# HenryHZY/VL-PET

Hardware: AMD Instinct MI355X
Metric: multitask samples/sec (BART-base, r=96) (higher is better)
Workload: dtype bf16

## Files before the change

include/vlpet_hip.h:

```cpp
#ifndef VLPET_HIP_H
#define VLPET_HIP_H
#include <stddef.h>
#include <stdint.h>

#ifdef __cplusplus
extern "C" {
#endif

#define VLPET_F32 0
#define VLPET_BF16 1

#define VLPET_E_SHAPE (-1)
#define VLPET_E_RANK (-2)
#define VLPET_E_ALIGN (-3)
#define VLPET_E_WORKSPACE (-4)
#define VLPET_E_NULL (-5)
#define VLPET_E_DTYPE (-6)
#define VLPET_E_ALIAS (-7)

#define VLPET_GATE_NONE 0
#define VLPET_GATE_MUL 1
#define VLPET_GATE_ADD 2

typedef void* vlpet_stream_t;
// ... 73 lines not shown
                                     float delta_scale, float x2_scale, float gate_scale,
                                     int io_dtype, vlpet_stream_t stream);

int vlpet_adapter_gate_bwd_saved_y(int phases, const void* dy, const void* x1, const void* x2, const void* y, const void* saved,
                                   const void* packed_a, const void* packed_g, const void* dx1_in, void* dx1, void* dx2,
                                   float* dwd, float* dbd, float* dwu, float* dbu,
                                   float* dwgd, float* dbgd, float* dwgu, float* dbgu,
                                   int r, int rg, void* workspace, size_t workspace_bytes,
                                   int64_t M, int d, int tiles, int gate_mode,
                                   float delta_scale, float x2_scale, float gate_scale,
                                   int io_dtype, vlpet_stream_t stream);

int vlpet_parallel_adapter_fwd(const void* x, const void* y, const void* packed, void* out,
                               int64_t M, int d, int tiles, float scale,
                               int io_dtype, vlpet_stream_t stream);
int vlpet_parallel_adapter_bwd(const void* dy, const void* x, const void* packed, void* dx,
                               float* dwd, float* dbd, float* dwu, float* dbu, int r,
                               void* workspace, size_t workspace_bytes,
                               int64_t M, int d, int tiles, float scale,
                               int io_dtype, vlpet_stream_t stream);

int vlpet_parallel_adapter_fwd_save(const void* x, const void* y, const void* packed, void* out, void* saved,
                                    int64_t M, int d, int tiles, float scale, int io_dtype, vlpet_stream_t stream);
int vlpet_parallel_adapter_bwd_saved(const void* dy, const void* x, const void* saved, const void* packed, void* dx,
                                     float* dwd, float* dbd, float* dwu, float* dbu, int r,
                                     void* workspace, size_t workspace_bytes, int64_t M, int d, int tiles,
                                     float scale, int io_dtype, vlpet_stream_t stream);

int vlpet_lora_delta_fwd(const void* x, const void* base, const void* packed,
                         const uint8_t* keep_mask, float p, uint64_t seed, uint8_t* keep_out, void* out,
                         int64_t M, int d, int tiles, float scaling,
                         int io_dtype, vlpet_stream_t stream);
int vlpet_lora_delta_bwd(const void* dy, const void* x, const void* packed,
                         const uint8_t* keep_mask, float p, uint64_t seed, void* dx,
                         float* da, float* db, int r,
                         void* workspace, size_t workspace_bytes,
                         int64_t M, int d, int tiles, float scaling,
                         int io_dtype, vlpet_stream_t stream);

size_t vlpet_lora_saved_bytes(int64_t M, int d, int tiles, int io_dtype);
int vlpet_lora_delta_fwd_save(const void* x, const void* base, const void* packed,
                              const uint8_t* keep_mask, float p, uint64_t seed, uint8_t* keep_out, void* out,
                              void* saved, int64_t M, int d, int tiles, float scaling,
                              int io_dtype, vlpet_stream_t stream);
int vlpet_lora_r8_applies(int64_t M, int d, int r, int io_dtype);
int vlpet_lora_delta_fwd_r8(const void* x, const void* base, const void* packed, const uint8_t* keep_mask, float p,
                            uint64_t seed, uint8_t* keep_out, void* out, void* saved, int64_t M, int d, int r,
                            float scaling, int io_dtype, vlpet_stream_t stream);
int vlpet_lora_delta_bwd_saved(const void* dy, const void* x, const void* saved, const void* packed,
                               const uint8_t* keep_mask, float p, uint64_t seed, void* dx,
                               float* da, float* db, int r,
                               void* workspace, size_t workspace_bytes,
                               int64_t M, int d, int tiles, float scaling,
                               int io_dtype, vlpet_stream_t stream);

size_t vlpet_visproj_packed_bytes(int d_out, int feat_dim, int io_dtype);
int vlpet_visproj_pack(const void* w, const void* b, int d_out, int feat_dim, int param_dtype, int io_dtype,
                       void* packed, vlpet_stream_t stream);
int vlpet_visproj_fwd(const void* feats, const void* packed, const float* gamma, const float* beta,
                      const void* r, void* out, void* xhat, float* rstd,
                      int64_t M, int feat_dim, int d_out, float eps, int rms,
                      int io_dtype, vlpet_stream_t stream);
size_t vlpet_visproj_gemm_workspace_bytes(int64_t M, int feat_dim, int d_out);
size_t vlpet_visproj_gemm_exchange_bytes(int d_out);
int vlpet_visproj_fwd_gemm(const void* feats, const void* w_io, const float* bias, const float* gamma, const float* beta,
                           const void* r, void* out, void* xhat, float* rstd, float* mean, void* workspace,
                           size_t workspace_bytes, int64_t M, int feat_dim, int d_out, float eps, int rms, int io_dtype,
                           vlpet_stream_t stream);
int vlpet_visproj_fwd_gemm_cfg(const void* feats, const void* w_io, const float* bias, const float* gamma, const float* beta,
                               const void* r, void* out, void* xhat, float* rstd, float* mean, void* workspace,
                               size_t workspace_bytes, int64_t M, int feat_dim, int d_out, float eps, int rms, int io_dtype,
                               int form, int rows_per_workgroup, vlpet_stream_t stream);
int vlpet_sum_n(const void* const* srcs, int n, void* out, int64_t len, int io_dtype, vlpet_stream_t stream);
int vlpet_vispos_applies(int d, int n_img);
int vlpet_vispos_fwd(const float* pos, const float* w, const float* b, const float* gamma, const float* beta,
                     const void* img_table, int img_table_dtype, int n_img, const int64_t* img_ids, int64_t img_ids_bstride,
                     const void* obj_table, int obj_table_dtype, int64_t obj_rows, const int64_t* obj_ids, int64_t obj_ids_bstride,
                     void* out, int64_t M, int N, int d, float eps, int rms, int io_dtype, vlpet_stream_t stream);
size_t vlpet_vispos_bwd_workspace_bytes(int64_t M, int d, int n_img);
int vlpet_vispos_bwd(const void* dout, const float* pos, const float* w, const float* b, const float* gamma,
                     int n_img, const int64_t* img_ids, int64_t img_ids_bstride,
                     float* dw, float* db, float* dgamma, float* dbeta, float* dimg,
                     void* workspace, size_t workspace_bytes, int64_t M, int N, int d, float eps, int rms, int io_dtype,
                     vlpet_stream_t stream);
size_t vlpet_visproj_wgrad_workspace_bytes(int64_t M, int feat_dim, int d_out);
size_t vlpet_visproj_wgrad_workspace_bytes_io(int64_t M, int feat_dim, int d_out, int io_dtype);
int vlpet_visproj_wgrad(const void* dpre, const void* feats, float* dw, float* db,
                        void* workspace, size_t workspace_bytes,
                        int64_t M, int feat_dim, int d_out, int io_dtype, vlpet_stream_t stream);

size_t vlpet_lowrank_packed_bytes(int tiles, int feat_dim, int d_out, int io_dtype);
int vlpet_lowrank_pack(const void* const* wd_heads, const void* const* bd_heads, int n_heads,
                       const void* wu, const void* bu, int r, int feat_dim, int d_out, int tiles,
                       int param_dtype, int io_dtype, void* packed, vlpet_stream_t stream);
int vlpet_lowrank_gate_fwd(const void* feats, const void* packed_a, const void* packed_g, void* fe,
                           void* saved, int64_t M, int feat_dim, int d_out, int tiles, int gate_residual,
                           int io_dtype, vlpet_stream_t stream);
size_t vlpet_lowrank_bwd_workspace_bytes(int64_t M, int feat_dim, int d_out, int tiles, int io_dtype);
int vlpet_lowrank_gate_bwd(const void* dfe, const void* feats, const void* saved, const void* packed_a,
                           const void* packed_g, float* dwd, float* dbd, float* dwu, float* dbu,
                           float* dwgd, float* dbgd, float* dwgu, float* dbgu, int r, int rg,
                           void* workspace, size_t workspace_bytes, int64_t M, int feat_dim, int d_out,
                           int tiles, int gate_residual, int io_dtype, vlpet_stream_t stream);
int vlpet_norm_residual_fwd(const void* y, const void* r, const float* gamma, const float* beta, void* out,
                            float* mean, float* rstd, int64_t M, int d, float eps, int io_dtype,
                            vlpet_stream_t stream);

int vlpet_sublayer_tail_partials(int64_t M);
int vlpet_sublayer_tail_fwd(const void* y, const void* x1, const float* gamma, const float* beta, void* out,
                            void* h_save, float* mean, float* rstd, uint8_t* keep_out, int64_t M, int d,
                            float eps, float p, uint64_t seed, int norm_mode, int io_dtype,
                            vlpet_stream_t stream);
int vlpet_sublayer_tail_bwd(const void* dout, const void* h_save, const float* mean, const float* rstd,
                            const float* gamma, void* dx1, void* dy, float* dgb_partials, int64_t M, int d,
                            float p, uint64_t seed, int norm_mode, int io_dtype, vlpet_stream_t stream);
int vlpet_sublayer_tail_bwd_out(const void* dout, const void* out_save, const float* rstd, const float* gamma, const float* beta,
                                void* dx1, void* dy, float* dgb_partials, int64_t M, int d,
                                float p, uint64_t seed, int io_dtype, vlpet_stream_t stream);
int vlpet_sublayer_tail_reduce(const float* dgb_partials, int n_partials, int d, float* dgamma, float* dbeta,
                               vlpet_stream_t stream);
int vlpet_colsum_partial(const void* x, int64_t M, int n, float* workspace, int io_dtype, vlpet_stream_t stream);
int vlpet_reduce_batch(const float* const* partials, float* const* out0, float* const* out1, const int* n_partials,
                       const int* d, int n_jobs, vlpet_stream_t stream);
int vlpet_rmsnorm_fwd(const void* x, const float* gamma, void* out, float* rstd, int64_t M, int d, float eps, int io_dtype,
                      vlpet_stream_t stream);
int vlpet_rmsnorm_bwd(const void* dout, const void* x, const float* rstd, const float* gamma, const void* dx_in, void* dx,
                      float* dgb_partials, int64_t M, int d, int io_dtype, vlpet_stream_t stream);
int vlpet_sublayer_tail_rms_fwd(const void* y, const void* x1, const float* gamma_next, void* sum, void* normed, float* rstd,
                                int64_t M, int d, float eps, float p, uint64_t seed, int io_dtype, vlpet_stream_t stream);
int vlpet_rmsnorm_tail_bwd(const void* d_normed, const void* sum, const float* rstd, const float* gamma_next, const void* dsum_in,
                           void* dx1, void* dy, float* dgb_partials, int64_t M, int d, float p, uint64_t seed, int io_dtype,
                           vlpet_stream_t stream);
int vlpet_colsum(const void* x, int64_t M, int n, float* workspace, float* out, int io_dtype, vlpet_stream_t stream);
int vlpet_layernorm_bwd_xhat(const void* dout, const void* xhat, const float* rstd, const float* gamma, void* dx,
                             float* dgb_partials, int64_t M, int d, int io_dtype, vlpet_stream_t stream);

#define VLPET_ACT_GELU 0
#define VLPET_ACT_GELU_NEW 1
#define VLPET_ACT_RELU 2
int vlpet_act_dropout_fwd(const void* x, void* out, uint8_t* keep_out, int64_t n, int act, float p, uint64_t seed,
                          int io_dtype, vlpet_stream_t stream);
int vlpet_act_dropout_bwd(const void* dy, const void* x, void* dx, int64_t n, int act, float p, uint64_t seed,
                          int io_dtype, vlpet_stream_t stream);
int vlpet_concat_dropout_fwd(const void* a, const void* v, void* x, int64_t B, int La, int Lv, int d, float p, uint64_t seed,
                             int io_dtype, vlpet_stream_t stream);
int vlpet_concat_dropout_bwd(const void* dx, void* da, void* dv, int64_t B, int La, int Lv, int d, float p, uint64_t seed,
                             int io_dtype, vlpet_stream_t stream);
int vlpet_prefix_concat_chunks(int64_t B);
size_t vlpet_prefix_concat_ws_bytes(int64_t B, int P, int d);
int vlpet_prefix_concat_dropout_fwd(const void* pre, const void* a, const void* v, void* x, int64_t B, int P, int La, int Lv, int d,
                                    float p, uint64_t seed, int io_dtype, vlpet_stream_t stream);
int vlpet_prefix_concat_dropout_bwd(const void* dx, void* dpre, void* da, void* dv, float* ws, int64_t B, int P, int La, int Lv, int d,
                                    float p, uint64_t seed, int io_dtype, vlpet_stream_t stream);

int vlpet_ce_loss_fwd(const void* logits, const int64_t* labels, float* loss, float* lse, int64_t N, int V, int ld,
                      int io_dtype, vlpet_stream_t stream);
int vlpet_ce_loss_bwd(const void* logits, const int64_t* labels, const float* lse, const float* dloss, void* dlogits,
                      int64_t N, int V, int ld, int io_dtype, vlpet_stream_t stream);
int vlpet_ce_loss_fwd_checked(const void* logits, const int64_t* labels, float* loss, float* lse, unsigned int* bad_count,
                              int64_t N, int V, int ld, int io_dtype, vlpet_stream_t stream);

#define VLPET_ATTN_MAX_LEN 128
int vlpet_attn_fwd(const void* q, const void* k, const void* v, const uint8_t* key_mask, void* o, float* lse, uint8_t* keep_out,
                   int B, int H, int Lq, int Lk, int causal, float scale, float p, uint64_t seed, vlpet_stream_t stream);
int vlpet_attn_bwd(const void* q, const void* k, const void* v, const void* o, const void* dout, const float* lse,
                   const uint8_t* key_mask, void* dq, void* dk, void* dv, int B, int H, int Lq, int Lk, int causal,
                   float scale, float p, uint64_t seed, vlpet_stream_t stream);
int vlpet_attn_fwd_ld(const void* q, const void* k, const void* v, const uint8_t* key_mask, void* o, float* lse, uint8_t* keep_out,
                      int B, int H, int Lq, int Lk, int ld_q, int ld_kv, int causal, float scale, float p, uint64_t seed,
                      vlpet_stream_t stream);
int vlpet_attn_bwd_ld(const void* q, const void* k, const void* v, const void* o, const void* dout, const float* lse,
                      const uint8_t* key_mask, void* dq, void* dk, void* dv, int B, int H, int Lq, int Lk, int ld_q, int ld_kv,
                      int causal, float scale, float p, uint64_t seed, vlpet_stream_t stream);
int vlpet_attn_fwd_bias(const void* q, const void* k, const void* v, const uint8_t* key_mask, const float* bias, void* o,
                        float* lse, uint8_t* keep_out, int B, int H, int Lq, int Lk, int ld_q, int ld_kv, int causal,
                        float scale, float p, uint64_t seed, vlpet_stream_t stream);
int vlpet_attn_bwd_bias(const void* q, const void* k, const void* v, const void* o, const void* dout, const float* lse,
                        const uint8_t* key_mask, const float* bias, const float* bias_t, void* dq, void* dk, void* dv,
                        int B, int H, int Lq, int Lk, int ld_q, int ld_kv, int causal, float scale, float p, uint64_t seed,
                        vlpet_stream_t stream);
int vlpet_attn_fwd_kv(const void* q, const void* k, const void* v, const uint8_t* key_mask, const float* bias, void* o,
                      float* lse, uint8_t* keep_out, int B, int H, int Lq, int Lk, int ld_q, int ld_k, int ld_v, int causal,
                      float scale, float p, uint64_t seed, vlpet_stream_t stream);
int vlpet_attn_bwd_kv(const void* q, const void* k, const void* v, const void* o, const void* dout, const float* lse,
                      const uint8_t* key_mask, const float* bias, const float* bias_t, void* dq, void* dk, void* dv,
                      int B, int H, int Lq, int Lk, int ld_q, int ld_k, int ld_v, int causal, float scale, float p, uint64_t seed,
                      vlpet_stream_t stream);
#define VLPET_ATTN_LONG_MAX_LEN 1024
int vlpet_attn_long_fwd(const void* q, const void* k, const void* v, const uint8_t* key_mask, const float* bias, void* o,
                        float* lse, int B, int H, int Lq, int Lk, int ld_q, int ld_k, int ld_v, int causal, float scale,
                        vlpet_stream_t stream);
int vlpet_attn_long_fwd_train(const void* q, const void* k, const void* v, const uint8_t* key_mask, const float* bias, void* o,
                              float* lse, uint8_t* keep_out, int B, int H, int Lq, int Lk, int ld_q, int ld_k, int ld_v, int causal,
                              float scale, float p, uint64_t seed, vlpet_stream_t stream);
int vlpet_attn_long_bwd(const void* q, const void* k, const void* v, const void* o, const void* dout, const float* lse,
                        const uint8_t* key_mask, const float* bias, const float* bias_t, void* dq, void* dk, void* dv,
                        int B, int H, int Lq, int Lk, int ld_q, int ld_k, int ld_v, int causal, float scale, float p, uint64_t seed,
                        float* delta, vlpet_stream_t stream);

int vlpet_downsample_fwd(const void* x, void* out, int64_t n_images, int s_in, int s_out, int dim,
                         int in_dtype, int out_dtype, vlpet_stream_t stream);

int vlpet_rowgate_partials(int64_t M);
int vlpet_row_dot(const void* a, const void* c, const float* wa, const float* wc, float* s_out, int64_t M, int d,
                  int io_dtype, vlpet_stream_t stream);
int vlpet_row_affine(const void* h, const float* alpha, const float* gamma, void* y, int64_t M, int d,
                     int io_dtype, vlpet_stream_t stream);
int vlpet_rowgate_bwd(const void* dy, const void* x1, const void* h, const float* alpha, const float* beta,
                      const float* wa, const float* wc, void* dh, void* dx1, float* partials, int64_t M, int d,
                      int io_dtype, vlpet_stream_t stream);
int vlpet_vecgate_fwd(const void* h, const float* v, const float* u, void* y, int64_t M, int d, int io_dtype,
                      vlpet_stream_t stream);
int vlpet_vecgate_bwd(const void* dy, const void* h, const float* v, void* dh, float* partials, int64_t M, int d,
                      int io_dtype, vlpet_stream_t stream);

int vlpet_optim_blocks(int64_t n);
int vlpet_grad_sumsq(const float* g, int64_t n, float* partials, vlpet_stream_t stream);
int vlpet_adamw_step(float* p, float* g, float* m, float* v, const uint8_t* decay_mask, int64_t n,
                     const float* partials, int n_partials, float max_norm, float grad_scale, float lr,
                     float beta1, float beta2, float eps, float weight_decay, int step, int variant,
                     int zero_grad, float* norm_out, vlpet_stream_t stream);

int vlpet_adamw_step_sliced(float* p, float* g, float* m, float* v, const uint8_t* decay_mask, int64_t n,
                            const float* partials, int n_partials, float max_norm, float grad_scale, float lr,
                            float beta1, float beta2, float eps, float weight_decay, const int32_t* slice_of,
                            const float* slice_bc, int variant, int zero_grad, float* norm_out,
                            vlpet_stream_t stream);

int vlpet_attn_decode(const void* q, int64_t ld_q, void* k_cache, void* v_cache, int64_t ld_k, int64_t bs_k, int64_t ld_v,
                      int64_t bs_v, const void* k_new, const void* v_new, int64_t ld_new, int pos, const uint8_t* key_mask,
                      int64_t ld_mask, const float* bias, int64_t ld_bias, void* o, int64_t ld_o, int B, int H, int D, int Lk,
                      float scale, int io_dtype, vlpet_stream_t stream);
int vlpet_greedy_pick(const void* logits, int64_t ld, int V, int64_t* ids, int64_t ld_ids, int pos, int* unfinished, int* counter,
                      int B, int eos_token_id, int pad_token_id, int min_length, int no_repeat_ngram_size, int io_dtype,
                      vlpet_stream_t stream);

int vlpet_attn_decode_beam(const void* q, int64_t ld_q, void* k_cache, void* v_cache, int64_t ld_k, int64_t bs_k, int64_t ld_v,
                           int64_t bs_v, const void* k_new, const void* v_new, int64_t ld_new, int pos, const uint8_t* key_mask,
                           int64_t ld_mask, const float* bias, int64_t ld_bias, void* o, int64_t ld_o, int B, int H, int D,
                           int Lk, float scale, int group, const int* key_rows, int64_t ld_key_rows, int io_dtype,
                           vlpet_stream_t stream);
int vlpet_beam_rows(const void* logits, int64_t ld, int V, const int64_t* ids, int64_t ld_ids, int pos, int rows, int num_beams,
                    int slices, int eos_token_id, int min_length, int no_repeat_ngram_size, int force_eos, float* part_stats,
                    float* part_val, int* part_tok, int io_dtype, vlpet_stream_t stream);
int vlpet_beam_advance(const float* part_stats, const float* part_val, const int* part_tok, int slices, int V, int B, int num_beams,
                       float* beam_scores, const int64_t* ids_in, int64_t* ids_out, int64_t ld_ids, const int* key_rows_in,
                       int* key_rows_out, int64_t ld_key_rows, int64_t* next_tokens, float* hyp_score, int* hyp_meta,
                       int64_t* hyp_tokens, int64_t ld_hyp, float* item_worst, int* item_state, int* counter, int pos,
                       int eos_token_id, int pad_token_id, float length_penalty, int early_stopping, vlpet_stream_t stream);

int vlpet_attn_decode_at(const void* q, int64_t ld_q, void* k_cache, void* v_cache, int64_t ld_k, int64_t bs_k, int64_t ld_v,
                         int64_t bs_v, const void* k_new, const void* v_new, int64_t ld_new, const int* pos_dev, int pos_limit,
                         const uint8_t* key_mask, int64_t ld_mask, const float* bias, int64_t ld_bias, int64_t pos_stride_bias,
                         void* o, int64_t ld_o, int B, int H, int D, int Lk, float scale, const int* key_rows,
                         int64_t ld_key_rows, int64_t parity_stride_key_rows, int io_dtype, vlpet_stream_t stream);
int vlpet_greedy_pick_at(const void* logits, int64_t ld, int V, int64_t* ids, int64_t ld_ids, const int* pos_dev, int pos_limit,
                         int* unfinished, int* counters, int64_t* next_tokens, int B, int eos_token_id, int pad_token_id,
                         int min_length, int no_repeat_ngram_size, int io_dtype, vlpet_stream_t stream);
int vlpet_beam_rows_at(const void* logits, int64_t ld, int V, const int64_t* ids, int64_t ld_ids, int64_t parity_stride_ids,
                       const int* pos_dev, int pos_limit, int rows, int num_beams, int slices, int eos_token_id, int min_length,
                       int no_repeat_ngram_size, int force_eos_pos, float* part_stats, float* part_val, int* part_tok,
                       int io_dtype, vlpet_stream_t stream);
int vlpet_beam_advance_at(const float* part_stats, const float* part_val, const int* part_tok, int slices, int V, int B,
                          int num_beams, float* beam_scores, int64_t* ids, int64_t ld_ids, int64_t parity_stride_ids,
                          int* key_rows, int64_t ld_key_rows, int64_t parity_stride_key_rows, int64_t* next_tokens,
                          float* hyp_score, int* hyp_meta, int64_t* hyp_tokens, int64_t ld_hyp, float* item_worst, int* item_state,
                          int* counters, const int* pos_dev, int pos_limit, int eos_token_id, int pad_token_id,
                          float length_penalty, int early_stopping, vlpet_stream_t stream);

int vlpet_adapter_tail_rows(void);
int vlpet_adapter_tail_applies(int64_t M, int d, int r, int io_dtype);
int vlpet_adapter_tail_fwd(const void* h, const void* res, const void* down_w, const void* down_b, const void* up_w,
                           const void* up_b, const float* gamma, const float* beta, void* out, int64_t M, int d, int r,
                           float scale, float eps, int norm_mode, int param_dtype, int io_dtype, vlpet_stream_t stream);

size_t vlpet_phm_workspace_bytes(int d, int r, int n);
int vlpet_phm_expand_pair_fwd(const void* rule_d, const void* W_d, const void* rule_u, const void* W_u, void* wt_d, void* wt_u,
                              int d, int r, int n, int param_dtype, vlpet_stream_t stream);
int vlpet_phm_expand_pair_bwd(const float* dwt_d, const float* dwt_u, const void* rule_d, const void* W_d, const void* rule_u,
                              const void* W_u, float* drule_d, float* dW_d, float* drule_u, float* dW_u, void* workspace,
                              size_t workspace_bytes, int d, int r, int n, int param_dtype, vlpet_stream_t stream);

#ifdef __cplusplus
}
#endif
#endif
```

vl-pet_amd/_lib.py:

```python
from __future__ import annotations

import ctypes
import os
from ctypes import c_char_p, c_float, c_int, c_int64, c_size_t, c_uint64, c_void_p

_HERE = os.path.dirname(os.path.abspath(__file__))
LIB_PATH = os.environ.get("VLPET_LIB") or os.path.join(_HERE, "lib", "libvlpet_hip.so")

VLPET_F32 = 0
VLPET_BF16 = 1
GATE_NONE, GATE_MUL, GATE_ADD = 0, 1, 2

_lib = None

SIGNATURES = {
    "vlpet_version": (c_int, []),
    "vlpet_error_string": (c_char_p, [c_int]),
    "vlpet_rank_tiles": (c_int, [c_int]),
    "vlpet_packed_bytes": (c_size_t, [c_int, c_int, c_int]),
    "vlpet_pack_pair": (c_int, [c_void_p, c_void_p, c_int, c_void_p, c_void_p, c_int, c_int, c_int, c_int, c_int,
                                c_void_p, c_void_p]),
    "vlpet_pack_pairs": (c_int, [c_int, c_void_p, c_void_p, c_int, c_void_p, c_void_p, c_int, c_int, c_int, c_int, c_int,
                                 c_void_p, c_void_p]),
    "vlpet_adapter_gate_fwd": (c_int, [c_void_p, c_void_p, c_void_p, c_void_p, c_void_p, c_int64, c_int, c_int,
                                       c_int, c_float, c_float, c_float, c_int, c_void_p]),
    "vlpet_saved_bytes": (c_size_t, [c_int64, c_int, c_int]),
    "vlpet_adapter_gate_fwd_save": (c_int, [c_void_p, c_void_p, c_void_p, c_void_p, c_void_p, c_void_p, c_int64, c_int,
                                            c_int, c_int, c_float, c_float, c_float, c_int, c_void_p]),
    "vlpet_adapter_gate_bwd_saved": (c_int, [c_int] + [c_void_p] * 8 + [c_void_p] * 8 + [c_int, c_int, c_void_p, c_size_t,
                                                                                        c_int64, c_int, c_int, c_int,
                                                                                        c_float, c_float, c_float, c_int,
                                                                                        c_void_p]),
    "vlpet_adapter_gate_bwd_saved_acc": (c_int, [c_int] + [c_void_p] * 9 + [c_void_p] * 8 + [c_int, c_int, c_void_p, c_size_t,
                                                                                            c_int64, c_int, c_int, c_int,
                                                                                            c_float, c_float, c_float, c_int,
                                                                                            c_void_p]),
    "vlpet_adapter_gate_bwd_saved_y": (c_int, [c_int] + [c_void_p] * 10 + [c_void_p] * 8 + [c_int, c_int, c_void_p, c_size_t,
                                                                                           c_int64, c_int, c_int, c_int,
                                                                                           c_float, c_float, c_float, c_int,
                                                                                           c_void_p]),
    "vlpet_bwd_workspace_bytes": (c_size_t, [c_int64, c_int, c_int, c_int, c_int]),
    "vlpet_adapter_gate_bwd_form": (c_int, [c_int64, c_int, c_int, c_int]),
    "vlpet_adapter_gate_bwd_finalize_launch": (c_int, [c_int64, c_int, c_int, c_int]),
    "vlpet_debug_build": (c_int, []),
    "vlpet_test_hold_cus": (c_int, [c_int, c_int, c_void_p, c_int, c_void_p]),
    "vlpet_set_seed_counter": (c_int, [c_void_p]),
    "vlpet_adapter_gate_bwd": (c_int, [c_void_p] * 7 + [c_void_p] * 8 + [c_int, c_int, c_void_p, c_size_t, c_int64,
                                                                         c_int, c_int, c_int, c_float, c_float,
                                                                         c_float, c_int, c_void_p]),
    "vlpet_adapter_gate_bwd_phase": (c_int, [c_int] + [c_void_p] * 7 + [c_void_p] * 8 + [c_int, c_int, c_void_p, c_size_t,
                                                                                        c_int64, c_int, c_int, c_int,
                                                                                        c_float, c_float, c_float, c_int,
                                                                                        c_void_p]),
    "vlpet_parallel_adapter_fwd": (c_int, [c_void_p, c_void_p, c_void_p, c_void_p, c_int64, c_int, c_int, c_float,
                                           c_int, c_void_p]),
    "vlpet_parallel_adapter_bwd": (c_int, [c_void_p] * 4 + [c_void_p] * 4 + [c_int, c_void_p, c_size_t, c_int64,
                                                                             c_int, c_int, c_float, c_int, c_void_p]),
    "vlpet_parallel_adapter_fwd_save": (c_int, [c_void_p, c_void_p, c_void_p, c_void_p, c_void_p, c_int64, c_int, c_int,
                                                c_float, c_int, c_void_p]),
    "vlpet_parallel_adapter_bwd_saved": (c_int, [c_void_p] * 5 + [c_void_p] * 4 + [c_int, c_void_p, c_size_t, c_int64,
                                                                                   c_int, c_int, c_float, c_int, c_void_p]),
    "vlpet_lora_delta_fwd": (c_int, [c_void_p, c_void_p, c_void_p, c_void_p, c_float, c_uint64, c_void_p, c_void_p,
                                     c_int64, c_int, c_int, c_float, c_int, c_void_p]),
    "vlpet_lora_saved_bytes": (c_size_t, [c_int64, c_int, c_int, c_int]),
    "vlpet_lora_delta_fwd_save": (c_int, [c_void_p, c_void_p, c_void_p, c_void_p, c_float, c_uint64, c_void_p, c_void_p,
                                          c_void_p, c_int64, c_int, c_int, c_float, c_int, c_void_p]),
    "vlpet_lora_r8_applies": (c_int, [c_int64, c_int, c_int, c_int]),
    "vlpet_lora_delta_fwd_r8": (c_int, [c_void_p, c_void_p, c_void_p, c_void_p, c_float, c_uint64, c_void_p, c_void_p,
                                        c_void_p, c_int64, c_int, c_int, c_float, c_int, c_void_p]),
    "vlpet_lora_delta_bwd_saved": (c_int, [c_void_p, c_void_p, c_void_p, c_void_p, c_void_p, c_float, c_uint64, c_void_p,
                                           c_void_p, c_void_p, c_int, c_void_p, c_size_t, c_int64, c_int, c_int, c_float,
                                           c_int, c_void_p]),
    "vlpet_visproj_packed_bytes": (c_size_t, [c_int, c_int, c_int]),
    "vlpet_visproj_pack": (c_int, [c_void_p, c_void_p, c_int, c_int, c_int, c_int, c_void_p, c_void_p]),
    "vlpet_visproj_fwd": (c_int, [c_void_p] * 8 + [c_int64, c_int, c_int, c_float, c_int, c_int, c_void_p]),
    "vlpet_visproj_gemm_workspace_bytes": (c_size_t, [c_int64, c_int, c_int]),
    "vlpet_visproj_gemm_exchange_bytes": (c_size_t, [c_int]),
    "vlpet_visproj_fwd_gemm": (c_int, [c_void_p] * 11 + [c_size_t, c_int64, c_int, c_int, c_float, c_int, c_int, c_void_p]),
    "vlpet_visproj_fwd_gemm_cfg": (c_int, [c_void_p] * 11 + [c_size_t, c_int64, c_int, c_int, c_float, c_int, c_int, c_int, c_int, c_void_p]),
    "vlpet_sum_n": (c_int, [c_void_p, c_int, c_void_p, c_int64, c_int, c_void_p]),
    "vlpet_vispos_applies": (c_int, [c_int, c_int]),
    "vlpet_vispos_fwd": (c_int, [c_void_p] * 5 + [c_void_p, c_int, c_int, c_void_p, c_int64] + [c_void_p, c_int, c_int64, c_void_p, c_int64]
                         + [c_void_p, c_int64, c_int, c_int, c_float, c_int, c_int, c_void_p]),
    "vlpet_vispos_bwd_workspace_bytes": (c_size_t, [c_int64, c_int, c_int]),
    "vlpet_vispos_bwd": (c_int, [c_void_p] * 5 + [c_int, c_void_p, c_int64] + [c_void_p] * 5
                         + [c_void_p, c_size_t, c_int64, c_int, c_int, c_float, c_int, c_int, c_void_p]),
    "vlpet_visproj_wgrad_workspace_bytes": (c_size_t, [c_int64, c_int, c_int]),
    "vlpet_visproj_wgrad_workspace_bytes_io": (c_size_t, [c_int64, c_int, c_int, c_int]),
    "vlpet_visproj_wgrad": (c_int, [c_void_p] * 5 + [c_size_t, c_int64, c_int, c_int, c_int, c_void_p]),
    "vlpet_lowrank_packed_bytes": (c_size_t, [c_int, c_int, c_int, c_int]),
    "vlpet_lowrank_pack": (c_int, [c_void_p, c_void_p, c_int, c_void_p, c_void_p] + [c_int] * 6 + [c_void_p, c_void_p]),
    "vlpet_lowrank_gate_fwd": (c_int, [c_void_p] * 5 + [c_int64] + [c_int] * 5 + [c_void_p]),
    "vlpet_lowrank_bwd_workspace_bytes": (c_size_t, [c_int64, c_int, c_int, c_int, c_int]),
    "vlpet_lowrank_gate_bwd": (c_int, [c_void_p] * 13 + [c_int, c_int, c_void_p, c_size_t, c_int64] + [c_int] * 5 + [c_void_p]),
    "vlpet_norm_residual_fwd": (c_int, [c_void_p] * 7 + [c_int64, c_int, c_float, c_int, c_void_p]),
    "vlpet_rowgate_partials": (c_int, [c_int64]),
    "vlpet_row_dot": (c_int, [c_void_p] * 5 + [c_int64, c_int, c_int, c_void_p]),
    "vlpet_row_affine": (c_int, [c_void_p] * 4 + [c_int64, c_int, c_int, c_void_p]),
    "vlpet_rowgate_bwd": (c_int, [c_void_p] * 10 + [c_int64, c_int, c_int, c_void_p]),
    "vlpet_vecgate_fwd": (c_int, [c_void_p] * 4 + [c_int64, c_int, c_int, c_void_p]),
    "vlpet_vecgate_bwd": (c_int, [c_void_p] * 5 + [c_int64, c_int, c_int, c_void_p]),
    "vlpet_optim_blocks": (c_int, [c_int64]),
    "vlpet_grad_sumsq": (c_int, [c_void_p, c_int64, c_void_p, c_void_p]),
    "vlpet_adamw_step": (c_int, [c_void_p] * 5 + [c_int64, c_void_p, c_int] + [c_float] * 7 + [c_int, c_int, c_int,
                                                                                           c_void_p, c_void_p]),
    "vlpet_adamw_step_sliced": (c_int, [c_void_p] * 5 + [c_int64, c_void_p, c_int] + [c_float] * 7 + [c_void_p, c_void_p,
                                                                                                  c_int, c_int, c_void_p,
                                                                                                  c_void_p]),
    "vlpet_downsample_fwd": (c_int, [c_void_p, c_void_p, c_int64, c_int, c_int, c_int, c_int, c_int, c_void_p]),
    "vlpet_sublayer_tail_partials": (c_int, [c_int64]),
    "vlpet_sublayer_tail_fwd": (c_int, [c_void_p] * 9 + [c_int64, c_int, c_float, c_float, c_uint64, c_int, c_int, c_void_p]),
    "vlpet_sublayer_tail_bwd": (c_int, [c_void_p] * 8 + [c_int64, c_int, c_float, c_uint64, c_int, c_int, c_void_p]),
    "vlpet_sublayer_tail_bwd_out": (c_int, [c_void_p] * 8 + [c_int64, c_int, c_float, c_uint64, c_int, c_void_p]),
    "vlpet_sublayer_tail_reduce": (c_int, [c_void_p, c_int, c_int, c_void_p, c_void_p, c_void_p]),
    "vlpet_layernorm_bwd_xhat": (c_int, [c_void_p] * 6 + [c_int64, c_int, c_int, c_void_p]),
    "vlpet_colsum": (c_int, [c_void_p, c_int64, c_int, c_void_p, c_void_p, c_int, c_void_p]),
    "vlpet_colsum_partial": (c_int, [c_void_p, c_int64, c_int, c_void_p, c_int, c_void_p]),
    "vlpet_reduce_batch": (c_int, [c_void_p, c_void_p, c_void_p, c_void_p, c_void_p, c_int, c_void_p]),
    "vlpet_rmsnorm_fwd": (c_int, [c_void_p] * 4 + [c_int64, c_int, c_float, c_int, c_void_p]),
    "vlpet_rmsnorm_bwd": (c_int, [c_void_p] * 7 + [c_int64, c_int, c_int, c_void_p]),
    "vlpet_sublayer_tail_rms_fwd": (c_int, [c_void_p] * 6 + [c_int64, c_int, c_float, c_float, c_uint64, c_int, c_void_p]),
    "vlpet_rmsnorm_tail_bwd": (c_int, [c_void_p] * 8 + [c_int64, c_int, c_float, c_uint64, c_int, c_void_p]),
    "vlpet_attn_fwd": (c_int, [c_void_p] * 7 + [c_int] * 5 + [c_float, c_float, c_uint64, c_void_p]),
    "vlpet_attn_bwd": (c_int, [c_void_p] * 10 + [c_int] * 5 + [c_float, c_float, c_uint64, c_void_p]),
    "vlpet_attn_fwd_ld": (c_int, [c_void_p] * 7 + [c_int] * 7 + [c_float, c_float, c_uint64, c_void_p]),
    "vlpet_attn_bwd_ld": (c_int, [c_void_p] * 10 + [c_int] * 7 + [c_float, c_float, c_uint64, c_void_p]),
    "vlpet_attn_fwd_bias": (c_int, [c_void_p] * 8 + [c_int] * 7 + [c_float, c_float, c_uint64, c_void_p]),
    "vlpet_attn_bwd_bias": (c_int, [c_void_p] * 12 + [c_int] * 7 + [c_float, c_float, c_uint64, c_void_p]),
    "vlpet_concat_dropout_fwd": (c_int, [c_void_p] * 3 + [c_int64, c_int, c_int, c_int, c_float, c_uint64, c_int, c_void_p]),
    "vlpet_concat_dropout_bwd": (c_int, [c_void_p] * 3 + [c_int64, c_int, c_int, c_int, c_float, c_uint64, c_int, c_void_p]),
    "vlpet_prefix_concat_chunks": (c_int, [c_int64]),
    "vlpet_prefix_concat_ws_bytes": (c_size_t, [c_int64, c_int, c_int]),
    "vlpet_prefix_concat_dropout_fwd": (c_int, [c_void_p] * 4 + [c_int64, c_int, c_int, c_int, c_int, c_float, c_uint64, c_int, c_void_p]),
    "vlpet_prefix_concat_dropout_bwd": (c_int, [c_void_p] * 5 + [c_int64, c_int, c_int, c_int, c_int, c_float, c_uint64, c_int, c_void_p]),
    "vlpet_attn_fwd_kv": (c_int, [c_void_p] * 8 + [c_int] * 8 + [c_float, c_float, c_uint64, c_void_p]),
    "vlpet_attn_bwd_kv": (c_int, [c_void_p] * 12 + [c_int] * 8 + [c_float, c_float, c_uint64, c_void_p]),
    "vlpet_attn_long_fwd": (c_int, [c_void_p] * 7 + [c_int] * 8 + [c_float, c_void_p]),
    "vlpet_attn_long_fwd_train": (c_int, [c_void_p] * 8 + [c_int] * 8 + [c_float, c_float, c_uint64, c_void_p]),
    "vlpet_attn_long_bwd": (c_int, [c_void_p] * 12 + [c_int] * 8 + [c_float, c_float, c_uint64, c_void_p, c_void_p]),
    "vlpet_ce_loss_fwd": (c_int, [c_void_p] * 4 + [c_int64, c_int, c_int, c_int, c_void_p]),
    "vlpet_ce_loss_fwd_checked": (c_int, [c_void_p] * 5 + [c_int64, c_int, c_int, c_int, c_void_p]),
    "vlpet_ce_loss_bwd": (c_int, [c_void_p] * 5 + [c_int64, c_int, c_int, c_int, c_void_p]),
    "vlpet_act_dropout_fwd": (c_int, [c_void_p] * 3 + [c_int64, c_int, c_float, c_uint64, c_int, c_void_p]),
    "vlpet_act_dropout_bwd": (c_int, [c_void_p] * 3 + [c_int64, c_int, c_float, c_uint64, c_int, c_void_p]),
    "vlpet_attn_decode": (c_int, [c_void_p, c_int64, c_void_p, c_void_p, c_int64, c_int64, c_int64, c_int64, c_void_p, c_void_p,
                                  c_int64, c_int, c_void_p, c_int64, c_void_p, c_int64, c_void_p, c_int64, c_int, c_int, c_int,
                                  c_int, c_float, c_int, c_void_p]),
    "vlpet_greedy_pick": (c_int, [c_void_p, c_int64, c_int, c_void_p, c_int64, c_int, c_void_p, c_void_p, c_int, c_int, c_int,
                                  c_int, c_int, c_int, c_void_p]),
    "vlpet_attn_decode_beam": (c_int, [c_void_p, c_int64, c_void_p, c_void_p, c_int64, c_int64, c_int64, c_int64, c_void_p,
                                       c_void_p, c_int64, c_int, c_void_p, c_int64, c_void_p, c_int64, c_void_p, c_int64, c_int,
                                       c_int, c_int, c_int, c_float, c_int, c_void_p, c_int64, c_int, c_void_p]),
    "vlpet_beam_rows": (c_int, [c_void_p, c_int64, c_int, c_void_p, c_int64, c_int, c_int, c_int, c_int, c_int, c_int, c_int, c_int,
                                c_void_p, c_void_p, c_void_p, c_int, c_void_p]),
    "vlpet_beam_advance": (c_int, [c_void_p, c_void_p, c_void_p, c_int, c_int, c_int, c_int, c_void_p, c_void_p, c_void_p, c_int64,
                                   c_void_p, c_void_p, c_int64, c_void_p, c_void_p, c_void_p, c_void_p, c_int64, c_void_p,
                                   c_void_p, c_void_p, c_int, c_int, c_int, c_float, c_int, c_void_p]),
    "vlpet_attn_decode_at": (c_int, [c_void_p, c_int64, c_void_p, c_void_p, c_int64, c_int64, c_int64, c_int64, c_void_p, c_void_p,
                                     c_int64, c_void_p, c_int, c_void_p, c_int64, c_void_p, c_int64, c_int64, c_void_p, c_int64,
                                     c_int, c_int, c_int, c_int, c_float, c_void_p, c_int64, c_int64, c_int, c_void_p]),
    "vlpet_greedy_pick_at": (c_int, [c_void_p, c_int64, c_int, c_void_p, c_int64, c_void_p, c_int, c_void_p, c_void_p, c_void_p,
                                     c_int, c_int, c_int, c_int, c_int, c_int, c_void_p]),
    "vlpet_beam_rows_at": (c_int, [c_void_p, c_int64, c_int, c_void_p, c_int64, c_int64, c_void_p, c_int, c_int, c_int, c_int, c_int,
                                   c_int, c_int, c_int, c_void_p, c_void_p, c_void_p, c_int, c_void_p]),
    "vlpet_beam_advance_at": (c_int, [c_void_p, c_void_p, c_void_p, c_int, c_int, c_int, c_int, c_void_p, c_void_p, c_int64, c_int64,
                                      c_void_p, c_int64, c_int64, c_void_p, c_void_p, c_void_p, c_void_p, c_int64, c_void_p,
                                      c_void_p, c_void_p, c_void_p, c_int, c_int, c_int, c_float, c_int, c_void_p]),
    "vlpet_adapter_tail_rows": (c_int, []),
    "vlpet_adapter_tail_applies": (c_int, [c_int64, c_int, c_int, c_int]),
    "vlpet_adapter_tail_fwd": (c_int, [c_void_p] * 9 + [c_int64, c_int, c_int, c_float, c_float, c_int, c_int, c_int, c_void_p]),
    "vlpet_lora_delta_bwd": (c_int, [c_void_p, c_void_p, c_void_p, c_void_p, c_float, c_uint64, c_void_p, c_void_p,
                                     c_void_p, c_int, c_void_p, c_size_t, c_int64, c_int, c_int, c_float, c_int,
                                     c_void_p]),
    "vlpet_phm_workspace_bytes": (c_size_t, [c_int, c_int, c_int]),
    "vlpet_phm_expand_pair_fwd": (c_int, [c_void_p] * 6 + [c_int, c_int, c_int, c_int, c_void_p]),
    "vlpet_phm_expand_pair_bwd": (c_int, [c_void_p] * 11 + [c_size_t, c_int, c_int, c_int, c_int, c_void_p]),
}


def load():
    global _lib
    if _lib is not None:
        return _lib
    if not os.path.exists(LIB_PATH):
        raise RuntimeError(
            f"vl-pet_amd: HIP library not found at {LIB_PATH}; run `python -c 'import __graft_entry__ as g; "
            f"g.build()'` (there is no CPU fallback for the PET hot path)")
    import torch
    if torch.cuda.is_available():
        torch.cuda.init()
    lib = ctypes.CDLL(LIB_PATH)
    for name, (res, args) in SIGNATURES.items():
        fn = getattr(lib, name)
        fn.restype = res
        fn.argtypes = args
    _lib = lib
    return lib


def check(code: int, what: str):
    if code != 0:
        msg = load().vlpet_error_string(code)
        raise RuntimeError(f"vl-pet_amd: {what} failed: {msg.decode() if msg else code} (code {code})")
```

vl-pet_amd/csrc/api.hip:

```cpp
#include <atomic>
#include "../../include/vlpet_hip.h"
#include "common.h"
#include "kernels.h"
#include <cmath>
#include <stdlib.h>
#include <stdio.h>
#include <vector>

#define VLPET_VERSION 680
#define VLPET_VERSION_R3 300
#define VLPET_VERSION_R2 221

static inline bool aligned16(const void* p) { return (reinterpret_cast<uintptr_t>(p) & 15) == 0; }
static inline size_t align256(size_t v) { return (v + 255) / 256 * 256; }
static inline int herr(hipError_t e) { return e == hipSuccess ? 0 : (int)e; }

extern "C" int vlpet_version(void) { return VLPET_VERSION; }
extern "C" int vlpet_debug_build(void) { return VLPET_IS_DEBUG_BUILD; }

__global__ __launch_bounds__(64) void hold_cus_kernel(unsigned* release, unsigned long long ticks) {
    extern __shared__ __attribute__((aligned(16))) uint8_t hold_smem[];
    typedef __attribute__((address_space(1))) unsigned gu32;
    if (threadIdx.x == 0) {
        hold_smem[0] = 1;
        const unsigned long long t0 = wall_clock64();
        while (__hip_atomic_load((gu32*)release, __ATOMIC_RELAXED, __HIP_MEMORY_SCOPE_AGENT) == 0u && wall_clock64() - t0 < ticks)
            __builtin_amdgcn_s_sleep(32);
    }
}
extern "C" int vlpet_test_hold_cus(int workgroups, int lds_bytes, void* release_flag, int max_ms, vlpet_stream_t stream) {
    if (!release_flag) return VLPET_E_NULL;
    if (workgroups <= 0 || workgroups > 1024 || lds_bytes < 0 || lds_bytes > 160 * 1024 || max_ms <= 0) return VLPET_E_SHAPE;
    if (max_ms > 10000) max_ms = 10000;
    hipError_t e = hipFuncSetAttribute(reinterpret_cast<const void*>(hold_cus_kernel), hipFuncAttributeMaxDynamicSharedMemorySize, lds_bytes);
    if (e != hipSuccess) return herr(e);
    hipLaunchKernelGGL(hold_cus_kernel, dim3((unsigned)workgroups), dim3(64), (size_t)lds_bytes, (hipStream_t)stream,
                       reinterpret_cast<unsigned*>(release_flag), (unsigned long long)max_ms * 100000ull);
    return herr(hipGetLastError());
}

extern "C" const char* vlpet_error_string(int code) {
    switch (code) {
        case 0: return "success";
        case VLPET_E_SHAPE: return "bad shape (need M > 0, d % 64 == 0, r > 0)";
        case VLPET_E_RANK: return "unsupported bottleneck rank (max 192) or tile count";
        case VLPET_E_ALIGN: return "pointer not 16-byte aligned";
        case VLPET_E_WORKSPACE: return "workspace too small";
        case VLPET_E_NULL: return "required pointer is NULL";
        case VLPET_E_DTYPE: return "unsupported dtype";
        case VLPET_E_ALIAS: return "output overlaps an input";
        default: return code > 0 ? hipGetErrorString((hipError_t)code) : "unknown error";
    }
}

extern "C" int vlpet_rank_tiles(int r) {
    if (r <= 0) return VLPET_E_SHAPE;
    if (r <= 32) return 1;
    if (r <= 96) return 3;
    if (r <= 192) return 6;
    return VLPET_E_RANK;
}

static inline bool tiles_ok(int t) { return t == 1 || t == 3 || t == 6; }
static inline bool dtype_ok(int t) { return t == VLPET_F32 || t == VLPET_BF16; }

extern "C" size_t vlpet_packed_bytes(int tiles, int d, int io_dtype) {
    return (size_t)pack_geom(tiles, d, io_dtype == VLPET_F32 ? 2 : 1).total_bytes;
}

extern "C" int vlpet_pack_pair(const void* const* wd_heads, const void* const* bd_heads, int n_heads,
                               const void* wu, const void* bu, int r, int d, int tiles,
                               int param_dtype, int io_dtype, void* packed, vlpet_stream_t stream) {
    if (!wd_heads || !wu || !packed) return VLPET_E_NULL;
    if (r <= 0 || d <= 0 || d % 64 != 0 || n_heads <= 0 || n_heads > VLPET_MAX_HEADS || r % n_heads != 0)
        return VLPET_E_SHAPE;
    if (!tiles_ok(tiles) || r > 32 * tiles) return VLPET_E_RANK;
    if (!dtype_ok(param_dtype) || !dtype_ok(io_dtype)) return VLPET_E_DTYPE;
    if (!aligned16(packed)) return VLPET_E_ALIGN;
    PackArgs a;
    for (int i = 0; i < VLPET_MAX_HEADS; ++i) {
        a.wd[i] = i < n_heads ? wd_heads[i] : nullptr;
        a.bd[i] = (bd_heads && i < n_heads) ? bd_heads[i] : nullptr;
        if (i < n_heads && a.wd[i] == nullptr) return VLPET_E_NULL;
    }
    a.wu = wu; a.bu = bu;
    a.n_heads = n_heads; a.rows_per_head = r / n_heads;
    a.r = r; a.d = d; a.RT = tiles; a.src_bf16 = param_dtype == VLPET_BF16;
    a.n_packs = 4;
    a.out = reinterpret_cast<uint8_t*>(packed);
    return herr(launch_pack_pair(a, io_dtype == VLPET_F32 ? 2 : 1, (hipStream_t)stream));
}

extern "C" int vlpet_pack_pairs(int n, const void* const* wd_heads_flat, const void* const* bd_heads_flat, int n_heads,
                                const void* const* wu, const void* const* bu, int r, int d, int tiles,
                                int param_dtype, int io_dtype, void* const* packed, vlpet_stream_t stream) {
    if (n <= 0) return 0;
    if (!wd_heads_flat || !wu || !packed) return VLPET_E_NULL;
    if (r <= 0 || d <= 0 || d % 64 != 0 || n_heads <= 0 || n_heads > VLPET_MAX_HEADS || r % n_heads != 0) return VLPET_E_SHAPE;
    if (!tiles_ok(tiles) || r > 32 * tiles) return VLPET_E_RANK;
    if (!dtype_ok(param_dtype) || !dtype_ok(io_dtype)) return VLPET_E_DTYPE;
    for (int i0 = 0; i0 < n; i0 += VLPET_PACK_BATCH) {
        PackBatch b;
        b.n = n - i0 < VLPET_PACK_BATCH ? n - i0 : VLPET_PACK_BATCH;
        for (int k = 0; k < b.n; ++k) {
            PackArgs& a = b.p[k];
            const int idx = i0 + k;
            for (int i = 0; i < VLPET_MAX_HEADS; ++i) {
                a.wd[i] = i < n_heads ? wd_heads_flat[(size_t)idx * n_heads + i] : nullptr;
                a.bd[i] = (bd_heads_flat && i < n_heads) ? bd_heads_flat[(size_t)idx * n_heads + i] : nullptr;
                if (i < n_heads && a.wd[i] == nullptr) return VLPET_E_NULL;
            }
            a.wu = wu[idx]; a.bu = bu ? bu[idx] : nullptr;
            if (!a.wu || !packed[idx]) return VLPET_E_NULL;
            if (!aligned16(packed[idx])) return VLPET_E_ALIGN;
            a.n_heads = n_heads; a.rows_per_head = r / n_heads;
            a.r = r; a.d = d; a.RT = tiles; a.src_bf16 = param_dtype == VLPET_BF16;
            a.n_packs = 4;
            a.out = reinterpret_cast<uint8_t*>(packed[idx]);
        }
        hipError_t e = launch_pack_pairs(b, io_dtype == VLPET_F32 ? 2 : 1, (hipStream_t)stream);
        if (e != hipSuccess) return (int)e;
    }
    return 0;
}

static int check_common(int64_t M, int d, int tiles, int io_dtype) {
    if (M <= 0 || d <= 0 || d % 64 != 0) return VLPET_E_SHAPE;
    if (!tiles_ok(tiles)) return VLPET_E_RANK;
    if (!dtype_ok(io_dtype)) return VLPET_E_DTYPE;
    return 0;
}

static int gate_flags(int gate_mode, int* flags) {
    *flags = 0;
    if (gate_mode == VLPET_GATE_MUL) *flags = PET_GATE;
    else if (gate_mode == VLPET_GATE_ADD) *flags = PET_GATE | PET_GATE_ADD;
    else if (gate_mode != VLPET_GATE_NONE) return VLPET_E_SHAPE;
    return 0;
}

static size_t saved_stride(int64_t M, int tiles, int io_dtype) {
    return align256((size_t)M * 32 * tiles * (io_dtype == VLPET_F32 ? 4 : 2));
}
extern "C" size_t vlpet_saved_bytes(int64_t M, int tiles, int io_dtype) {
    if (M <= 0 || !tiles_ok(tiles)) return 0;
    return 4 * saved_stride(M, tiles, io_dtype);
}

static const DropSpec NO_DROP = {nullptr, nullptr, nullptr, nullptr, 0, 0, 1.f, nullptr};

static std::atomic<const uint64_t*> g_seed_ctr{nullptr};
extern "C" int vlpet_set_seed_counter(const uint64_t* device_counter) {
    g_seed_ctr.store(device_counter);
    return 0;
}

static bool k1_in_launch_reduce(int64_t M) {
    return M >= 8192;
}

static int make_drop(const uint8_t* keep_mask, float p, uint64_t seed, uint8_t* keep_out, DropSpec* ds) {
    if (!(p >= 0.f && p < 1.f)) return VLPET_E_SHAPE;
// ... 1155 lines not shown
                              uint8_t* keep_out, int B, int H, int Lq, int Lk, int causal, float scale, float p, uint64_t seed,
                              vlpet_stream_t stream) {
    return vlpet_attn_fwd_ld(q, k, v, key_mask, o, lse, keep_out, B, H, Lq, Lk, H * 64, H * 64, causal, scale, p, seed, stream);
}

extern "C" int vlpet_attn_bwd_kv(const void* q, const void* k, const void* v, const void* o, const void* dout, const float* lse,
                                 const uint8_t* key_mask, const float* bias, const float* bias_t, void* dq, void* dk, void* dv,
                                 int B, int H, int Lq, int Lk, int ld_q, int ld_k, int ld_v, int causal, float scale, float p, uint64_t seed,
                                 vlpet_stream_t stream) {
    AttnArgs a;
    int rc = attn_args(a, VLPET_ATTN_MAX_LEN, true, q, k, v, key_mask, bias, bias_t, o, lse, nullptr, dout, dq, dk, dv, nullptr,
                       B, H, Lq, Lk, ld_q, ld_k, ld_v, causal, scale, p, seed);
    return rc ? rc : herr(launch_attn(a, true, (hipStream_t)stream));
}
extern "C" int vlpet_attn_bwd_bias(const void* q, const void* k, const void* v, const void* o, const void* dout, const float* lse,
                                   const uint8_t* key_mask, const float* bias, const float* bias_t, void* dq, void* dk, void* dv,
                                   int B, int H, int Lq, int Lk, int ld_q, int ld_kv, int causal, float scale, float p, uint64_t seed,
                                   vlpet_stream_t stream) {
    return vlpet_attn_bwd_kv(q, k, v, o, dout, lse, key_mask, bias, bias_t, dq, dk, dv, B, H, Lq, Lk, ld_q, ld_kv, ld_kv, causal, scale, p, seed,
                             stream);
}

extern "C" int vlpet_attn_bwd_ld(const void* q, const void* k, const void* v, const void* o, const void* dout, const float* lse,
                                 const uint8_t* key_mask, void* dq, void* dk, void* dv, int B, int H, int Lq, int Lk, int ld_q,
                                 int ld_kv, int causal, float scale, float p, uint64_t seed, vlpet_stream_t stream) {
    return vlpet_attn_bwd_bias(q, k, v, o, dout, lse, key_mask, nullptr, nullptr, dq, dk, dv, B, H, Lq, Lk, ld_q, ld_kv, causal, scale, p, seed,
                               stream);
}

extern "C" int vlpet_attn_bwd(const void* q, const void* k, const void* v, const void* o, const void* dout, const float* lse,
                              const uint8_t* key_mask, void* dq, void* dk, void* dv, int B, int H, int Lq, int Lk, int causal,
                              float scale, float p, uint64_t seed, vlpet_stream_t stream) {
    return vlpet_attn_bwd_ld(q, k, v, o, dout, lse, key_mask, dq, dk, dv, B, H, Lq, Lk, H * 64, H * 64, causal, scale, p, seed, stream);
}

static int ce_common(int64_t N, int V, int ld, int io_dtype) {
    if (N <= 0 || V <= 0 || ld < V || (ld & 7) != 0) return VLPET_E_SHAPE;
    if (io_dtype != VLPET_F32 && io_dtype != VLPET_BF16) return VLPET_E_DTYPE;
    return 0;
}

extern "C" int vlpet_ce_loss_fwd_checked(const void* logits, const int64_t* labels, float* loss, float* lse, unsigned int* bad_count,
                                         int64_t N, int V, int ld, int io_dtype, vlpet_stream_t stream) {
    int rc = ce_common(N, V, ld, io_dtype);
    if (rc) return rc;
    if (!logits || !labels || !loss || !lse) return VLPET_E_NULL;
    if (!aligned16(logits)) return VLPET_E_ALIGN;
    CeArgs a{};
    a.logits = logits; a.labels = labels; a.loss = loss; a.lse = lse; a.dloss = nullptr; a.dlogits = nullptr;
    a.N = N; a.V = V; a.ld = ld; a.bad = bad_count;
    return herr(launch_ce(a, false, io_dtype == VLPET_F32, (hipStream_t)stream));
}
extern "C" int vlpet_ce_loss_fwd(const void* logits, const int64_t* labels, float* loss, float* lse, int64_t N, int V, int ld,
                                 int io_dtype, vlpet_stream_t stream) {
    return vlpet_ce_loss_fwd_checked(logits, labels, loss, lse, nullptr, N, V, ld, io_dtype, stream);
}

extern "C" int vlpet_ce_loss_bwd(const void* logits, const int64_t* labels, const float* lse, const float* dloss, void* dlogits,
                                 int64_t N, int V, int ld, int io_dtype, vlpet_stream_t stream) {
    int rc = ce_common(N, V, ld, io_dtype);
    if (rc) return rc;
    if (!logits || !labels || !lse || !dloss || !dlogits) return VLPET_E_NULL;
    if (!aligned16(logits) || !aligned16(dlogits)) return VLPET_E_ALIGN;
    CeArgs a{};
    a.logits = logits; a.labels = labels; a.loss = nullptr; a.lse = const_cast<float*>(lse); a.dloss = dloss; a.dlogits = dlogits;
    a.N = N; a.V = V; a.ld = ld;
    return herr(launch_ce(a, true, io_dtype == VLPET_F32, (hipStream_t)stream));
}

static int act_common(int64_t n, int act, float p, int io_dtype) {
    if (n <= 0 || (n & 7) != 0) return VLPET_E_SHAPE;
    if (act != VLPET_ACT_GELU && act != VLPET_ACT_GELU_NEW && act != VLPET_ACT_RELU) return VLPET_E_SHAPE;
    if (!(p >= 0.0f && p < 1.0f)) return VLPET_E_SHAPE;
    if (io_dtype != VLPET_F32 && io_dtype != VLPET_BF16) return VLPET_E_DTYPE;
    return 0;
}

extern "C" int vlpet_act_dropout_fwd(const void* x, void* out, uint8_t* keep_out, int64_t n, int act, float p, uint64_t seed,
                                     int io_dtype, vlpet_stream_t stream) {
    int rc = act_common(n, act, p, io_dtype);
    if (rc) return rc;
    if (!x || !out) return VLPET_E_NULL;
    if (!aligned16(x) || !aligned16(out)) return VLPET_E_ALIGN;
    ActDropArgs a{};
    a.x = x; a.dy = nullptr; a.out = out; a.keep_out = keep_out; a.n = n; a.act = act; a.thr = tail_thr(p);
    a.keep_scale = a.thr ? 1.0f / (1.0f - p) : 1.0f; a.seed = seed; a.seed_ctr = g_seed_ctr.load();
    return herr(launch_act_dropout(a, false, io_dtype == VLPET_F32, (hipStream_t)stream));
}

extern "C" int vlpet_concat_dropout_fwd(const void* a, const void* v, void* x, int64_t B, int La, int Lv, int d, float p, uint64_t seed,
                                        int io_dtype, vlpet_stream_t stream) {
    if (!a || !v || !x) return VLPET_E_NULL;
    if (B <= 0 || La <= 0 || Lv <= 0 || d <= 0 || d % 8 != 0 || !(p >= 0.f && p < 1.f)) return VLPET_E_SHAPE;
    if (!dtype_ok(io_dtype)) return VLPET_E_DTYPE;
    if (!aligned16(a) || !aligned16(v) || !aligned16(x)) return VLPET_E_ALIGN;
    const uint32_t thr = tail_thr(p);
    return herr(launch_cat_dropout(a, v, x, B, La, Lv, d, thr, thr ? 1.0f / (1.0f - p) : 1.0f, seed, g_seed_ctr.load(), false,
                                   io_dtype == VLPET_F32, (hipStream_t)stream));
}
extern "C" int vlpet_concat_dropout_bwd(const void* dx, void* da, void* dv, int64_t B, int La, int Lv, int d, float p, uint64_t seed,
                                        int io_dtype, vlpet_stream_t stream) {
    if (!dx || (!da && !dv)) return VLPET_E_NULL;
    if (B <= 0 || La <= 0 || Lv <= 0 || d <= 0 || d % 8 != 0 || !(p >= 0.f && p < 1.f)) return VLPET_E_SHAPE;
    if (!dtype_ok(io_dtype)) return VLPET_E_DTYPE;
    if (!aligned16(dx) || (da && !aligned16(da)) || (dv && !aligned16(dv))) return VLPET_E_ALIGN;
    const uint32_t thr = tail_thr(p);
    return herr(launch_cat_dropout(da, dv, const_cast<void*>(dx), B, La, Lv, d, thr, thr ? 1.0f / (1.0f - p) : 1.0f, seed, g_seed_ctr.load(), true,
                                   io_dtype == VLPET_F32, (hipStream_t)stream));
}

extern "C" int vlpet_prefix_concat_chunks(int64_t B) {
    if (B <= 0) return 0;
    int cs, nc;
    prefix_cat_split(B, &cs, &nc);
    return nc;
}
extern "C" size_t vlpet_prefix_concat_ws_bytes(int64_t B, int P, int d) {
    if (B <= 0 || P <= 0 || d <= 0) return 0;
    return (size_t)vlpet_prefix_concat_chunks(B) * (size_t)P * (size_t)d * sizeof(float);
}
static int prefix_cat_common(int64_t B, int P, int La, int Lv, int d, float p, int io_dtype) {
    if (B <= 0 || P <= 0 || La <= 0 || Lv <= 0 || d <= 0 || d % 8 != 0 || !(p >= 0.f && p < 1.f)) return VLPET_E_SHAPE;
    if (!dtype_ok(io_dtype)) return VLPET_E_DTYPE;
    return 0;
}
static PrefixCatArgs prefix_cat_args(const void* pre, const void* a, const void* v, void* x, int64_t B, int P, int La, int Lv, int d, float p,
                                     uint64_t seed) {
    PrefixCatArgs c{};
    c.pre = pre; c.a = a; c.v = v; c.x = x; c.B = B; c.P = P; c.La = La; c.Lv = Lv; c.d = d;
    prefix_cat_split(B, &c.CS, &c.NC);
    c.thr = tail_thr(p); c.keep_scale = c.thr ? 1.0f / (1.0f - p) : 1.0f; c.seed = seed; c.seed_ctr = g_seed_ctr.load();
    return c;
}
extern "C" int vlpet_prefix_concat_dropout_fwd(const void* pre, const void* a, const void* v, void* x, int64_t B, int P, int La, int Lv, int d,
                                               float p, uint64_t seed, int io_dtype, vlpet_stream_t stream) {
    if (!pre || !a || !v || !x) return VLPET_E_NULL;
    if (int rc = prefix_cat_common(B, P, La, Lv, d, p, io_dtype)) return rc;
    if (!aligned16(pre) || !aligned16(a) || !aligned16(v) || !aligned16(x)) return VLPET_E_ALIGN;
    const PrefixCatArgs c = prefix_cat_args(pre, a, v, x, B, P, La, Lv, d, p, seed);
    return herr(launch_prefix_cat(c, false, io_dtype == VLPET_F32, (hipStream_t)stream));
}
extern "C" int vlpet_prefix_concat_dropout_bwd(const void* dx, void* dpre, void* da, void* dv, float* ws, int64_t B, int P, int La, int Lv,
                                               int d, float p, uint64_t seed, int io_dtype, vlpet_stream_t stream) {
    if (!dx || (!dpre && !da && !dv) || (dpre && !ws)) return VLPET_E_NULL;
    if (int rc = prefix_cat_common(B, P, La, Lv, d, p, io_dtype)) return rc;
    if (!dpre && ws) return VLPET_E_SHAPE;
    if (!aligned16(dx) || (dpre && !aligned16(dpre)) || (da && !aligned16(da)) || (dv && !aligned16(dv)) || (ws && !aligned16(ws)))
        return VLPET_E_ALIGN;
    PrefixCatArgs c = prefix_cat_args(nullptr, da, dv, const_cast<void*>(dx), B, P, La, Lv, d, p, seed);
    c.dpre = dpre; c.ws = ws;
    return herr(launch_prefix_cat(c, true, io_dtype == VLPET_F32, (hipStream_t)stream));
}

extern "C" int vlpet_act_dropout_bwd(const void* dy, const void* x, void* dx, int64_t n, int act, float p, uint64_t seed,
                                     int io_dtype, vlpet_stream_t stream) {
    int rc = act_common(n, act, p, io_dtype);
    if (rc) return rc;
    if (!dy || !x || !dx) return VLPET_E_NULL;
    if (!aligned16(dy) || !aligned16(x) || !aligned16(dx)) return VLPET_E_ALIGN;
    ActDropArgs a{};
    a.x = x; a.dy = dy; a.out = dx; a.keep_out = nullptr; a.n = n; a.act = act; a.thr = tail_thr(p);
    a.keep_scale = a.thr ? 1.0f / (1.0f - p) : 1.0f; a.seed = seed; a.seed_ctr = g_seed_ctr.load();
    return herr(launch_act_dropout(a, true, io_dtype == VLPET_F32, (hipStream_t)stream));
}

extern "C" int vlpet_downsample_fwd(const void* x, void* out, int64_t n_images, int s_in, int s_out, int dim,
                                    int in_dtype, int out_dtype, vlpet_stream_t stream) {
    if (!x || !out) return VLPET_E_NULL;
    if (n_images <= 0 || s_in <= 0 || s_out <= 0 || s_out > s_in || dim <= 0 || dim % 8 != 0) return VLPET_E_SHAPE;
    if (!dtype_ok(in_dtype) || !dtype_ok(out_dtype)) return VLPET_E_DTYPE;
    if (!aligned16(x) || !aligned16(out)) return VLPET_E_ALIGN;
    PoolArgs a;
    a.x = x; a.out = out; a.n_img = n_images; a.s_in = s_in; a.s_out = s_out; a.dim = dim;
    return herr(launch_downsample(a, in_dtype == VLPET_F32, out_dtype == VLPET_F32, (hipStream_t)stream));
}

static int row_common(int64_t M, int d, int io_dtype) {
    if (M <= 0 || d <= 0 || d % 8 != 0) return VLPET_E_SHAPE;
    if (!dtype_ok(io_dtype)) return VLPET_E_DTYPE;
    if (d / (io_dtype == VLPET_F32 ? 4 : 8) > 4 * 64) return VLPET_E_SHAPE;
    return 0;
}
static int row_launch(RowArgs& a, int op, int64_t M, int d, int io_dtype, vlpet_stream_t stream) {
    a.M = M; a.d = d;
    return herr(launch_rowgate(a, op, io_dtype == VLPET_F32, (hipStream_t)stream));
}

extern "C" int vlpet_rowgate_partials(int64_t M) { return M > 0 ? rowgate_blocks(M) : 0; }

extern "C" int vlpet_row_dot(const void* a, const void* c, const float* wa, const float* wc, float* s_out, int64_t M,
                             int d, int io_dtype, vlpet_stream_t stream) {
    int rc = row_common(M, d, io_dtype);
    if (rc) return rc;
    if (!a || !s_out) return VLPET_E_NULL;
    if (!wa && !c) return VLPET_E_NULL;
    if (wa && c && !wc) return VLPET_E_NULL;
    if (!aligned16(a) || (c && !aligned16(c))) return VLPET_E_ALIGN;
    RowArgs r{};
    r.a = a; r.c = c; r.va = wa; r.vc = wc; r.rs = s_out;
    return row_launch(r, ROW_DOT, M, d, io_dtype, stream);
}

extern "C" int vlpet_row_affine(const void* h, const float* alpha, const float* gamma, void* y, int64_t M, int d,
                                int io_dtype, vlpet_stream_t stream) {
    int rc = row_common(M, d, io_dtype);
    if (rc) return rc;
    if (!h || !alpha || !y) return VLPET_E_NULL;
    if (!aligned16(h) || !aligned16(y)) return VLPET_E_ALIGN;
    RowArgs r{};
    r.a = h; r.ra = alpha; r.rb = gamma; r.o1 = y;
    return row_launch(r, ROW_AFFINE, M, d, io_dtype, stream);
}

extern "C" int vlpet_rowgate_bwd(const void* dy, const void* x1, const void* h, const float* alpha, const float* beta,
                                 const float* wa, const float* wc, void* dh, void* dx1, float* partials, int64_t M,
                                 int d, int io_dtype, vlpet_stream_t stream) {
    int rc = row_common(M, d, io_dtype);
    if (rc) return rc;
    if (!dy || !x1 || !h || !alpha || !beta || !wa || !wc || !dh || !dx1 || !partials) return VLPET_E_NULL;
    if (!aligned16(dy) || !aligned16(x1) || !aligned16(h) || !aligned16(dh) || !aligned16(dx1)) return VLPET_E_ALIGN;
    RowArgs r{};
    r.a = dy; r.c = x1; r.e = h; r.ra = alpha; r.rb = beta; r.va = wa; r.vc = wc; r.o1 = dh; r.o2 = dx1; r.part = partials;
    return row_launch(r, ROW_BWD, M, d, io_dtype, stream);
}

extern "C" int vlpet_vecgate_fwd(const void* h, const float* v, const float* u, void* y, int64_t M, int d, int io_dtype,
                                 vlpet_stream_t stream) {
    int rc = row_common(M, d, io_dtype);
    if (rc) return rc;
    if (!h || !v || !y) return VLPET_E_NULL;
    if (!aligned16(h) || !aligned16(y)) return VLPET_E_ALIGN;
    RowArgs r{};
    r.a = h; r.va = v; r.vc = u; r.o1 = y;
    return row_launch(r, VEC_FWD, M, d, io_dtype, stream);
}

extern "C" int vlpet_vecgate_bwd(const void* dy, const void* h, const float* v, void* dh, float* partials, int64_t M,
                                 int d, int io_dtype, vlpet_stream_t stream) {
    int rc = row_common(M, d, io_dtype);
    if (rc) return rc;
    if (!dy || !h || !v || !dh || !partials) return VLPET_E_NULL;
    if (!aligned16(dy) || !aligned16(h) || !aligned16(dh)) return VLPET_E_ALIGN;
    RowArgs r{};
    r.a = dy; r.c = h; r.va = v; r.o1 = dh; r.part = partials;
    return row_launch(r, VEC_BWD, M, d, io_dtype, stream);
}

extern "C" int vlpet_optim_blocks(int64_t n) { return n > 0 ? optim_blocks(n) : 0; }

extern "C" int vlpet_grad_sumsq(const float* g, int64_t n, float* partials, vlpet_stream_t stream) {
    if (!g || !partials) return VLPET_E_NULL;
    if (n <= 0) return VLPET_E_SHAPE;
    if (!aligned16(g)) return VLPET_E_ALIGN;
    return herr(launch_sumsq(g, n, partials, (hipStream_t)stream));
}

extern "C" int vlpet_adamw_step(float* p, float* g, float* m, float* v, const uint8_t* decay_mask, int64_t n,
                                const float* partials, int n_partials, float max_norm, float grad_scale, float lr,
                                float beta1, float beta2, float eps, float weight_decay, int step, int variant,
                                int zero_grad, float* norm_out, vlpet_stream_t stream) {
    if (!p || !g || !m || !v || !partials) return VLPET_E_NULL;
    if (n <= 0 || n_partials <= 0 || step <= 0 || (variant != 0 && variant != 1)) return VLPET_E_SHAPE;
    if (!aligned16(p) || !aligned16(g) || !aligned16(m) || !aligned16(v) || (decay_mask && ((uintptr_t)decay_mask & 3)))
        return VLPET_E_ALIGN;
    AdamwArgs a;
    a.p = p; a.g = g; a.m = m; a.v = v; a.decay = decay_mask; a.n = n; a.partials = partials; a.n_partials = n_partials;
    a.max_norm = max_norm; a.grad_scale = grad_scale; a.lr = lr; a.beta1 = beta1; a.beta2 = beta2; a.eps = eps;
    a.weight_decay = weight_decay;
    a.bias_c1 = (float)(1.0 - pow((double)beta1, (double)step));
    a.bias_c2_sqrt = (float)sqrt(1.0 - pow((double)beta2, (double)step));
    a.decay_first = variant == 1; a.eps_scaled = variant == 1; a.zero_grad = zero_grad; a.norm_out = norm_out;
    a.slice_of = nullptr; a.slice_bc = nullptr;
    return herr(launch_adamw(a, (hipStream_t)stream));
}

extern "C" int vlpet_adamw_step_sliced(float* p, float* g, float* m, float* v, const uint8_t* decay_mask, int64_t n,
                                       const float* partials, int n_partials, float max_norm, float grad_scale, float lr,
                                       float beta1, float beta2, float eps, float weight_decay, const int32_t* slice_of,
                                       const float* slice_bc, int variant, int zero_grad, float* norm_out,
                                       vlpet_stream_t stream) {
    if (!p || !g || !m || !v || !partials || !slice_of || !slice_bc) return VLPET_E_NULL;
    if (n <= 0 || n_partials <= 0 || (variant != 0 && variant != 1)) return VLPET_E_SHAPE;
    if (!aligned16(p) || !aligned16(g) || !aligned16(m) || !aligned16(v) || !aligned16(slice_of) ||
        (decay_mask && ((uintptr_t)decay_mask & 3)))
        return VLPET_E_ALIGN;
    AdamwArgs a;
    a.p = p; a.g = g; a.m = m; a.v = v; a.decay = decay_mask; a.n = n; a.partials = partials; a.n_partials = n_partials;
    a.max_norm = max_norm; a.grad_scale = grad_scale; a.lr = lr; a.beta1 = beta1; a.beta2 = beta2; a.eps = eps;
    a.weight_decay = weight_decay; a.bias_c1 = 1.f; a.bias_c2_sqrt = 1.f;
    a.decay_first = variant == 1; a.eps_scaled = variant == 1; a.zero_grad = zero_grad; a.norm_out = norm_out;
    a.slice_of = slice_of; a.slice_bc = slice_bc;
    return herr(launch_adamw(a, (hipStream_t)stream));
}

extern "C" int vlpet_adapter_tail_rows(void) { return adapter_tail_rows(); }

extern "C" int vlpet_adapter_tail_applies(int64_t M, int d, int r, int io_dtype) {
    return (M > 0 && (M + adapter_tail_rows() - 1) / adapter_tail_rows() <= 0x7fffffffLL && adapter_tail_geometry_ok(d, r) && dtype_ok(io_dtype)) ? 1 : 0;
}

static inline bool ranges_overlap(const void* a, const void* b, size_t bytes) {
    const uintptr_t x = reinterpret_cast<uintptr_t>(a), y = reinterpret_cast<uintptr_t>(b);
    return x < y + bytes && y < x + bytes;
}

extern "C" int vlpet_adapter_tail_fwd(const void* h, const void* res, const void* down_w, const void* down_b, const void* up_w,
// ... 82 lines not shown
```

vl-pet_amd/csrc/kernels.h:

```cpp
#pragma once
#include <cstdlib>
#include <hip/hip_runtime.h>
#include <stdint.h>
#include "rng.h"
#include "tuning.h"

#define VLPET_MAX_HEADS 16

struct PackArgs {
    const void* wd[VLPET_MAX_HEADS];
    const void* bd[VLPET_MAX_HEADS];
    const void* wu;
    const void* bu;
    int n_heads, rows_per_head;
    int r, d, RT;
    int src_bf16;
    int n_packs;
    uint8_t* out;
};
hipError_t launch_pack_pair(const PackArgs& a, int NS, hipStream_t stream);
#define VLPET_PACK_BATCH 8
struct PackBatch { PackArgs p[VLPET_PACK_BATCH]; int n; };
hipError_t launch_pack_pairs(const PackBatch& b, int NS, hipStream_t stream);

// ... 200 lines not shown
    int img_tab_bf16, obj_tab_bf16;
    const int64_t* img_ids; const int64_t* obj_ids;
    int64_t img_bstride, obj_bstride;
    int n_img; int64_t obj_rows;
    void* out;
    const void* dout;
    float* partial;
    float* dw; float* db; float* dgamma; float* dbeta; float* dimg;
    int64_t M; int N, d; float eps; int rms;
};
bool vispos_applies(int d, int n_img);
size_t vispos_bwd_workspace_bytes(int64_t M, int d, int n_img);
hipError_t launch_vispos_fwd(const VisPosArgs& a, int io_fp32, hipStream_t stream);
hipError_t launch_vispos_bwd(const VisPosArgs& a, int io_fp32, hipStream_t stream);

struct TailArgs {
    const void* y;
    const void* x1;
    void* out;
    void* h;
    const float* gamma;
    const float* beta;
    float* mean;
    float* rstd;
    uint8_t* keep_out;
    float* dgb;
    int64_t M;
    int d;
    float eps;
    uint32_t thr;
    float keep_scale;
    uint64_t seed;
    const uint64_t* seed_ctr;
    int norm;
    int post;
    int h_xhat;
    int h_out;
    const void* dres;
    int rms;
    void* out2;
    const float* gamma2;
};
hipError_t launch_tail(const TailArgs& a, int io_fp32, bool bwd, hipStream_t stream);
int tail_blocks(int64_t M);

struct Lora8Args {
    const void* x; const void* base; void* out;
    const uint8_t* pk;
    DropSpec drop;
    void* save;
    int64_t M; int d;
    float scaling;
};
bool lora8_applies(int64_t M, int d, int r, int io_fp32);
hipError_t launch_lora8_fwd(const Lora8Args& a, hipStream_t stream);
hipError_t launch_tail_reduce(const float* part, int nb, int d, float* dgamma, float* dbeta, hipStream_t stream);
hipError_t launch_colsum(const void* x, int64_t M, int n, float* part, float* out, int io_fp32, hipStream_t stream);
hipError_t launch_colsum_partial(const void* x, int64_t M, int n, float* part, int io_fp32, hipStream_t stream);
struct ReduceJob { const float* part; float* out0; float* out1; int nb; int d; };
#define VLPET_REDUCE_BATCH 96
struct ReduceBatch { ReduceJob j[VLPET_REDUCE_BATCH]; int n; };
hipError_t launch_tail_reduce_batch(const ReduceBatch& b, int max_d, hipStream_t stream);

struct PoolArgs {
    const void* x;
    void* out;
    int64_t n_img;
    int s_in, s_out, dim;
};
hipError_t launch_downsample(const PoolArgs& a, int in_fp32, int out_fp32, hipStream_t stream);

enum RowOp { ROW_DOT = 0, ROW_AFFINE = 1, ROW_BWD = 2, VEC_FWD = 3, VEC_BWD = 4 };
struct RowArgs {
    const void* a;
    const void* c;
    const void* e;
    void* o1;
    void* o2;
    const float* va;
    const float* vc;
    const float* ra;
    const float* rb;
    float* rs;
    float* part;
    int64_t M;
    int d;
};
hipError_t launch_rowgate(const RowArgs& a, int op, int io_fp32, hipStream_t stream);
int rowgate_blocks(int64_t M);

struct AdamwArgs {
    float* p; float* g; float* m; float* v;
    const uint8_t* decay;
    int64_t n;
    const float* partials; int n_partials;
    float max_norm;
    float grad_scale;
    float lr, beta1, beta2, eps, weight_decay;
    float bias_c1, bias_c2_sqrt;
    int decay_first;
    int eps_scaled;
    int zero_grad;
    float* norm_out;
    const int32_t* slice_of;
    const float* slice_bc;
};
hipError_t launch_add_inplace(void* dst, const void* src, int64_t n, int io_fp32, hipStream_t stream);
struct SumNArgs { const void* src[8]; void* out; };
hipError_t launch_sum_n(const SumNArgs& a, int n, int64_t len, int io_fp32, hipStream_t stream);
hipError_t launch_sumsq(const float* g, int64_t n, float* partials, hipStream_t stream);
hipError_t launch_adamw(const AdamwArgs& a, hipStream_t stream);
int optim_blocks(int64_t n);

inline int pick_row_groups(int64_t M, int max_rg, int min_rg) {
    if (const int rg = vlpet_tuning().rg; rg >= min_rg && rg <= max_rg && rg > 0) return rg;
    int best = max_rg;
    int64_t best_cost = -1;
    for (int rg = max_rg; rg >= min_rg; --rg) {
        const int64_t wgs = (M + 32 * rg - 1) / (32 * rg);
        const int64_t cost = ((wgs + 255) / 256) * (rg + 1);
        if (best_cost < 0 || cost < best_cost) { best = rg; best_cost = cost; }
    }
    return best;
}

#define VLPET_ACT_GELU 0
#define VLPET_ACT_GELU_NEW 1
#define VLPET_ACT_RELU 2
struct ActDropArgs {
    const void* x;
    const void* dy;
    void* out;
    uint8_t* keep_out;
    int64_t n;
    int act;
    uint32_t thr;
    float keep_scale;
    uint64_t seed;
    const uint64_t* seed_ctr;
};
hipError_t launch_act_dropout(const ActDropArgs& a, bool bwd, int io_fp32, hipStream_t stream);
hipError_t launch_cat_dropout(const void* a, const void* v, void* x, int64_t B, int La, int Lv, int d, uint32_t thr, float keep_scale,
                              uint64_t seed, const uint64_t* seed_ctr, bool bwd, int io_fp32, hipStream_t stream);
#define PREFIX_CAT_MAX_CHUNKS 32
struct PrefixCatArgs {
    const void* pre; const void* a; const void* v; void* x;
    void* dpre; float* ws;
    int64_t B; int P, La, Lv, d, CS, NC;
    uint32_t thr; float keep_scale; uint64_t seed; const uint64_t* seed_ctr;
};
void prefix_cat_split(int64_t B, int* cs, int* nc);
hipError_t launch_prefix_cat(const PrefixCatArgs& c, bool bwd, int io_fp32, hipStream_t stream);

struct CeArgs {
    const void* logits;
    const int64_t* labels;
    float* loss;
    float* lse;
    const float* dloss;
    void* dlogits;
    int64_t N;
    int V, ld;
    unsigned int* bad;
};
hipError_t launch_ce(const CeArgs& a, bool bwd, int io_fp32, hipStream_t stream);

struct AttnArgs {
    const __bf16* q; const __bf16* k; const __bf16* v;
    __bf16* o;
    float* lse;
    const __bf16* dout;
    __bf16* dq; __bf16* dk; __bf16* dv;
    const uint8_t* key_mask;
    const float* bias;
    const float* bias_t;
    uint8_t* keep_out;
    int B, H, Lq, Lk, causal;
    int ld_q, ld_kv;
    int ld_v;
    float scale;
    uint32_t thr;
    float inv_keep;
    uint64_t seed;
    const uint64_t* seed_ctr;
    int dbg;
};
size_t attn_lds_bytes(int Lq, int Lk, int bwd);
hipError_t launch_attn(const AttnArgs& a, bool bwd, hipStream_t stream);
hipError_t launch_attn_bwd_fewq(const AttnArgs& a, hipStream_t stream);
hipError_t launch_attn_long_fwd(const AttnArgs& a, hipStream_t stream);
hipError_t launch_attn_long_bwd(const AttnArgs& a, float* delta, hipStream_t stream);

struct AdapterTailArgs {
    const void* h;
    const void* res;
    const void* wd;
    const void* bd;
    const void* wu;
    const void* bu;
    const float* gamma;
    const float* beta;
    void* out;
    int64_t M;
    int d, r;
    float scale, eps;
    int norm;
};
int adapter_tail_rows(void);
bool adapter_tail_geometry_ok(int d, int r);
hipError_t launch_adapter_tail(const AdapterTailArgs& a, int io_fp32, int param_fp32, hipStream_t stream);

struct PhmLayer {
    const void* rule;
    const void* W;
    void* wt;
    const float* dwt;
    float* drule;
    float* dW;
    int in, out;
};
struct PhmArgs {
    PhmLayer l[2];
    int n;
    float* ws;
};
int64_t phm_layer_tiles(int in, int out, int n);
hipError_t launch_phm_expand_fwd(const PhmArgs& a, int param_fp32, hipStream_t stream);
hipError_t launch_phm_expand_bwd(const PhmArgs& a, int param_fp32, hipStream_t stream);
```

vl-pet_amd/host/bart.py:

```python
from __future__ import annotations

import copy
import math
from types import SimpleNamespace

import torch
import torch.nn as nn
import torch.nn.functional as F

from .. import attention as A
from .. import decode as D
from .. import functional as VF
from .. import adapter_tail as AT
from ..adapters import AdapterController
from ..encoder_pet import apply_pet, build_pet, has_pet
from ..lora import LoRALinearController, LoraConfig
from ..visual import Downsample, LowRankVisualEmbedding, VisualEmbedding
from ..prompt import PromptController
from .common import (COMPACTER_DEFAULTS, PROMPT_DEFAULTS, check_sequential_adapter_flags, derived_weights, eval_no_grad, fused_adapter_tail,
                     install_shared_phm_rule, is_key_mask, make_adapter_config, make_prompt_config, sequential_adapters, shift_right, unpack_vis_inputs,
                     value_parallel_adapter)

TASKS = ["vqa", "gqa", "nlvr", "caption"]

# ... 247 lines not shown
                k_slot = None
                if k_pre is not None:
                    (k, k_slot), v = k_pre, VF.linear_acc(src, kv_link, self.v_proj)
                else:
                    k, v = VF.linear_acc(src, kv_link, self.k_proj, self.v_proj)
                if self.attn_value_parallel_adapter is not None:
                    v = self.attn_value_parallel_adapter(src, task, y=v, link=kv_link)
                out = attention_core(q, k, v, self.num_heads, attn_mask, causal, self.dropout, self.training, k_slot=k_slot)
                return _linear(self.out_proj, out)
            v = _linear(self.v_proj, src)
            k = _linear(self.k_proj, src)
        if kv is not None and self.attn_value_parallel_adapter is not None:
            v = self.attn_value_parallel_adapter(src, task, y=v)
        out = attention_core(q, k, v, self.num_heads, attn_mask, causal, self.dropout, self.training)
        return _linear(self.out_proj, out)


    def _step_qkv(self, x, task):
        if self.use_lora:
            return self.q_proj(x, task)[:, 0], _linear(self.k_proj, x)[:, 0], self.v_proj(x, task)[:, 0]
        if FUSE_QKV:
            w, b = self._fused_qkv(x.dtype)
            qkv = F.linear(x[:, 0], w, b)
            E = self.embed_dim
            return qkv[:, :E], qkv[:, E:2 * E], qkv[:, 2 * E:]
        return _linear(self.q_proj, x)[:, 0], _linear(self.k_proj, x)[:, 0], _linear(self.v_proj, x)[:, 0]

    def step_self(self, x, k_cache, v_cache, pos, task=None, key_rows=None, pos_dev=None):
        q, k, v = self._step_qkv(x, task)
        out = D.decode_attention(q, k_cache, v_cache, self.num_heads, pos=pos, k_new=k, v_new=v, scale=self.head_dim ** -0.5,
                                 key_rows=key_rows, pos_dev=pos_dev)
        return _linear(self.out_proj, out[:, None])

    def cross_values(self, enc, task=None):
        v = self.v_proj(enc, task) if self.use_lora else _linear(self.v_proj, enc)
        if self.attn_value_parallel_adapter is not None:
            v = self.attn_value_parallel_adapter(enc, task, y=v)
        return v

    def step_cross(self, x, k_cache, v_cache, key_mask, task=None, group=1):
        q = self.q_proj(x, task) if self.use_lora else _linear(self.q_proj, x)
        out = D.decode_attention(q[:, 0], k_cache, v_cache, self.num_heads, key_mask=key_mask, scale=self.head_dim ** -0.5,
                                 group=group)
        return _linear(self.out_proj, out[:, None])


class BartEncoderLayer(nn.Module):
    def __init__(self, config):
        super().__init__()
        self.config = config
        d = config.d_model
        self.embed_dim = d
        self.self_attn = BartAttention(config, d, config.encoder_attention_heads, config.attention_dropout)
        self.self_attn_layer_norm = HostLayerNorm(d)
        self.dropout, self.activation_dropout = config.dropout, config.activation_dropout
        self.fc1 = nn.Linear(d, config.encoder_ffn_dim)
        self.fc2 = nn.Linear(config.encoder_ffn_dim, d)
        self.final_layer_norm = HostLayerNorm(d)
        build_pet(self, config, d, ("attn", "ff"))
        self.attn_adapter = self.ff_adapter = None
        if sequential_adapters(config, "encoder"):
            self.attn_adapter = AdapterController(config.adapter_config)
            self.ff_adapter = AdapterController(config.adapter_config)
        self.pet_config = copy.copy(config)
        self.pet_config.use_encoder_adapter_scaling = False
        self.pet_config.use_encoder_x2_scaling = False

    def forward(self, hidden, attn_mask=None, task=None):
        residual = hidden
        gl = _new_gemm_link(hidden)
        h = self.self_attn(hidden, attn_mask=attn_mask, task=task, in_link=gl)
        if self.attn_adapter is not None:
            hidden = _adapter_then_tail(self.attn_adapter, task, residual, h, self.self_attn_layer_norm, self.dropout, self.training, gl)
        elif has_pet(self, "attn"):
            hidden = _pet_then_tail(self, "attn", residual, h, self.self_attn_layer_norm, self.dropout, self.training,
                                    self.pet_config, gemm_link=gl)
        else:
            hidden = _tail_linked(residual, h, self.self_attn_layer_norm, self.dropout, self.training, gl)
        residual = hidden
        gl = _new_gemm_link(hidden)
        h = ffn_activation(_first_linear(self.fc1, hidden, gl), "gelu", self.activation_dropout, self.training)
        h = _linear(self.fc2, h)
        if self.ff_adapter is not None:
            return _adapter_then_tail(self.ff_adapter, task, residual, h, self.final_layer_norm, self.dropout, self.training, gl)
        if has_pet(self, "ff"):
            return _pet_then_tail(self, "ff", residual, h, self.final_layer_norm, self.dropout, self.training, self.pet_config,
                                  gemm_link=gl)
        return _tail_linked(residual, h, self.final_layer_norm, self.dropout, self.training, gl)


class BartDecoderLayer(nn.Module):
    def __init__(self, config):
        super().__init__()
        self.config = config
        d = config.d_model
        self.self_attn = BartAttention(config, d, config.decoder_attention_heads, config.attention_dropout)
        self.self_attn_layer_norm = HostLayerNorm(d)
        vpa = bool(config.use_decoder_enc_attn_value_parallel_adapter_down_dim) and not config.use_lora
        self.encoder_attn = BartAttention(config, d, config.decoder_attention_heads, config.attention_dropout,
                                          is_cross=True, value_adapter=vpa)
        self.encoder_attn_layer_norm = HostLayerNorm(d)
        self.dropout, self.activation_dropout = config.dropout, config.activation_dropout
        self.fc1 = nn.Linear(d, config.decoder_ffn_dim)
        self.fc2 = nn.Linear(config.decoder_ffn_dim, d)
        self.final_layer_norm = HostLayerNorm(d)
        self.self_attn_adapter = self.enc_attn_adapter = self.ff_adapter = None
        if sequential_adapters(config, "decoder"):
            self.self_attn_adapter = AdapterController(config.adapter_config)
            if config.add_adapter_cross_attn:
                self.enc_attn_adapter = AdapterController(config.adapter_config)
            self.ff_adapter = AdapterController(config.adapter_config)

    def _tail(self, ctl, task, residual, h, norm, gl=None):
        if ctl is not None:
            return _adapter_then_tail(ctl, task, residual, h, norm, self.dropout, self.training, gl)
        return _tail_linked(residual, h, norm, self.dropout, self.training, gl)

    def forward(self, hidden, enc, enc_mask=None, task=None, k_pre=None):
        residual = hidden
        gl = _new_gemm_link(hidden)
        h = self.self_attn(hidden, causal=True, task=task, in_link=gl)
        hidden = self._tail(self.self_attn_adapter, task, residual, h, self.self_attn_layer_norm, gl)
        residual = hidden
        gl = _new_gemm_link(hidden)
        h = self.encoder_attn(hidden, kv=enc, attn_mask=enc_mask, task=task, in_link=gl, k_pre=k_pre)
        hidden = self._tail(self.enc_attn_adapter, task, residual, h, self.encoder_attn_layer_norm, gl)
        residual = hidden
        gl = _new_gemm_link(hidden)
        h = ffn_activation(_first_linear(self.fc1, hidden, gl), "gelu", self.activation_dropout, self.training)
        h = _linear(self.fc2, h)
        return self._tail(self.ff_adapter, task, residual, h, self.final_layer_norm, gl)


    def step(self, x, cache, pos, state, task=None):
        ks, vs, kx, vx = cache
        kr, pd = state.key_rows, state.pos_dev
        h = self.self_attn.step_self(x, ks, vs, pos, task, key_rows=kr if kr is None or pd is not None else kr[pos & 1], pos_dev=pd)
        x = self._tail(self.self_attn_adapter, task, x, h, self.self_attn_layer_norm)
        h = self.encoder_attn.step_cross(x, kx, vx, state.key_mask, task, group=state.group)
        x = self._tail(self.enc_attn_adapter, task, x, h, self.encoder_attn_layer_norm)
        h = ffn_activation(_linear(self.fc1, x), "gelu", self.activation_dropout, self.training)
        return self._tail(self.ff_adapter, task, x, _linear(self.fc2, h), self.final_layer_norm)


class LearnedPositionalEmbedding(nn.Embedding):

    def __init__(self, num, dim):
        super().__init__(num + 2, dim)

    def forward(self, L: int, device):
        return super().forward(torch.arange(2, L + 2, device=device))


class JointEncoder(nn.Module):
    def __init__(self, config, embed_tokens):
        super().__init__()
        self.config = config
        d = config.d_model
        self.dropout = config.dropout
        self.embed_scale = math.sqrt(d) if config.scale_embedding else 1.0
        self.embed_tokens = embed_tokens
        self.embed_positions = LearnedPositionalEmbedding(config.max_position_embeddings, d)
        self.layers = nn.ModuleList([BartEncoderLayer(config) for _ in range(config.encoder_layers)])
        self.layernorm_embedding = HostLayerNorm(d)
        vis_cls = LowRankVisualEmbedding if getattr(config, "use_lowrank_visual_projector", False) else VisualEmbedding
        self.visual_embedding = vis_cls(config, self.embed_tokens)
        self.downsample = None
        if config.downsample:
            s = int(config.n_boxes ** 0.5)
            self.downsample = Downsample((s, s))
        if getattr(config, "encoder_prompt_config", None) is not None:
            self.prompt_modules = PromptController(config.encoder_prompt_config)

    def forward(self, input_ids, vis_inputs, attention_mask=None, task=None, no_padding=False):
        if getattr(self, "prompt_modules", None) is not None:
            return self._forward_prompted(input_ids, vis_inputs, attention_mask, task, no_padding)
        B, L = input_ids.shape
        if attention_mask is None and not no_padding:
            attention_mask = input_ids.ne(self.config.pad_token_id)
        x = self.embed_tokens(input_ids) * self.embed_scale + self.embed_positions(L, input_ids.device)
        vis = self.visual_embedding(*unpack_vis_inputs(vis_inputs, self.downsample, x.dtype)).to(x.dtype)
        if self.config.share_vis_lang_layer_norm:
            x = self.layernorm_embedding(torch.cat([x, vis], dim=1))
            x = F.dropout(x, p=self.dropout, training=self.training)
        else:
            from ..act import concat_dropout
            x = concat_dropout(self.layernorm_embedding(x), vis, self.dropout, self.training)
        mask = None
        if attention_mask is not None:
            full = torch.cat([attention_mask.bool(), torch.ones(B, vis.shape[1], dtype=torch.bool,
                                                                device=x.device)], dim=1)
            mask = full[:, None, None, :]
        for layer in self.layers:
            x = layer(x, mask, task)
        return x, mask

    def _forward_prompted(self, input_ids, vis_inputs, attention_mask, task, no_padding):
        B, L = input_ids.shape
        if attention_mask is None and not no_padding:
            attention_mask = input_ids.ne(self.config.pad_token_id)
        x = self.embed_tokens(input_ids) * self.embed_scale + self.embed_positions(L, input_ids.device)
        vis = self.visual_embedding(*unpack_vis_inputs(vis_inputs, self.downsample, x.dtype)).to(x.dtype)
        pre = self.prompt_modules.prompt_rows(task).to(x.dtype)
        P = pre.shape[0]
        if self.config.share_vis_lang_layer_norm:
            x = self.layernorm_embedding(torch.cat([pre.expand(B, -1, -1), x, vis], dim=1))
            x = F.dropout(x, p=self.dropout, training=self.training)
        else:
            from ..act import prefix_concat_dropout
            x = prefix_concat_dropout(self.layernorm_embedding(pre), self.layernorm_embedding(x), vis, self.dropout, self.training)
        mask = None
        if attention_mask is not None:
            ones = lambda n: torch.ones(B, n, dtype=torch.bool, device=x.device)
            mask = torch.cat([ones(P), attention_mask.bool(), ones(vis.shape[1])], dim=1)[:, None, None, :]
        for layer in self.layers:
            x = layer(x, mask, task)
        return x, mask


class BartDecoder(nn.Module):
    def __init__(self, config, embed_tokens):
        super().__init__()
        d = config.d_model
        self.dropout = config.dropout
        self.embed_scale = math.sqrt(d) if config.scale_embedding else 1.0
        self.embed_tokens = embed_tokens
        self.embed_positions = LearnedPositionalEmbedding(config.max_position_embeddings, d)
        self.layers = nn.ModuleList([BartDecoderLayer(config) for _ in range(config.decoder_layers)])
        self.layernorm_embedding = HostLayerNorm(d)

    def forward(self, input_ids, enc, enc_mask=None, task=None):
        B, L = input_ids.shape
        x = self.embed_tokens(input_ids) * self.embed_scale + self.embed_positions(L, input_ids.device)
        x = F.dropout(self.layernorm_embedding(x), p=self.dropout, training=self.training)
        n = len(self.layers)
        fused_keys = self._cross_keys_ok(enc, enc_mask)
        encs = VF.fanout(enc, n + (1 if fused_keys else 0))
        ks = self._cross_keys(encs[n]) if fused_keys else None
        for i, (layer, e) in enumerate(zip(self.layers, encs)):
            x = layer(x, e, enc_mask, task, k_pre=None if ks is None else (ks[0][i], None if ks[1] is None else (ks[1], i)))
        return x

    def _cross_keys_ok(self, enc, enc_mask) -> bool:
        if not FUSE_CROSS_KEYS or EAGER_ATTENTION or len(self.layers) < 2 or not enc.is_cuda or enc.dtype != torch.bfloat16:
            return False
        a0 = self.layers[0].encoder_attn
        if _route(enc.shape[1], enc.shape[1], a0.dropout, self.training, grad=True) is None or a0.head_dim != A.HEAD_DIM:
            return False
        if enc_mask is not None and not is_key_mask(enc_mask):
            return False
        return all((not l.encoder_attn.use_lora) and _frozen(l.encoder_attn.k_proj, l.encoder_attn.v_proj) for l in self.layers)

    def _cross_keys(self, enc):
        w, b = derived_weights(self, "_ck_cache", [l.encoder_attn.k_proj for l in self.layers], enc.dtype)
        return VF.cross_key_blocks(enc, w, b, len(self.layers))


    def init_cache(self, enc, key_mask, task, max_length, num_beams=1):
        if FUSE_CROSS_KEYS and not EAGER_ATTENTION and len(self.layers) >= 2 and enc.is_cuda:
            ks = self._cross_keys(enc)[0]
        else:
            ks = [_linear(l.encoder_attn.k_proj, enc) for l in self.layers]
        vs = [l.encoder_attn.cross_values(enc, task) for l in self.layers]
        return D.new_decode_state(enc, enc.shape[2], max_length, ks, vs, key_mask, num_beams)

    def step(self, tok, pos, state, task=None):
        if state.pos_dev is not None:
            p = self.embed_positions.weight[2:].index_select(0, state.pos_dev)
        else:
            p = self.embed_positions.weight[pos + 2]
        x = self.embed_tokens(tok)[:, None] * self.embed_scale + p
        x = F.dropout(self.layernorm_embedding(x), p=self.dropout, training=self.training)
        for layer, c in zip(self.layers, state.layers):
            x = layer.step(x, c, pos, state, task)
        return x[:, 0]


class VLBartModel(nn.Module):
    def __init__(self, config):
        super().__init__()
        self.shared = nn.Embedding(config.vocab_size, config.d_model, padding_idx=config.pad_token_id)
        self.encoder = JointEncoder(config, self.shared)
        self.decoder = BartDecoder(config, self.shared)


shift_tokens_right = shift_right


class VLBart(nn.Module):

    def __init__(self, config):
        super().__init__()
        self.config = config
        self.model = VLBartModel(config)
        self.register_buffer("final_logits_bias", torch.zeros(1, config.vocab_size))
        install_shared_phm_rule(self, [self.model], config.adapter_config)
        self.apply(self._init_weights)
        self.register_load_state_dict_post_hook(lambda module, incompatible: VF.invalidate_caches())

    def _init_weights(self, m):
        std = self.config.init_std
        if isinstance(m, nn.Linear):
            m.weight.data.normal_(0.0, std)
            if m.bias is not None:
                m.bias.data.zero_()
        elif isinstance(m, nn.Embedding):
            m.weight.data.normal_(0.0, std)
            if m.padding_idx is not None:
                m.weight.data[m.padding_idx].zero_()
        if isinstance(m, LoRALinearController):
            for t in m.tasks:
                nn.init.zeros_(m.lora_Bs[t])

    def _logits_bias(self):
        b = self.final_logits_bias
        key = (b.data_ptr(), b._version, VF.FROZEN_EPOCH)
        if getattr(self, "_bias_key", None) != key:
            self._bias_key, self._bias_nonzero = key, bool(b.any())
        return b if self._bias_nonzero else None

    def forward(self, input_ids, vis_inputs, labels, task, attention_mask=None, no_padding=False):
        cfg = self.config
        enc, mask = self.model.encoder(input_ids, vis_inputs, attention_mask, task, no_padding)
        dec_in = shift_tokens_right(labels, cfg.pad_token_id, cfg.decoder_start_token_id)
        h = self.model.decoder(dec_in, enc, mask, task)
        return lm_loss(h, self.model.shared.weight, labels, self._logits_bias())

    def generate(self, input_ids, vis_inputs, task, attention_mask=None, max_length=20, min_length=0, no_repeat_ngram_size=0,
                 eos_token_id=None, pad_token_id=None, no_padding=False, num_beams=1, length_penalty=1.0, early_stopping=False,
                 graph=False):
        from ..lmloss import _padded_head
        cfg = self.config
        eos = getattr(cfg, "eos_token_id", 2) if eos_token_id is None else eos_token_id
        pad = cfg.pad_token_id if pad_token_id is None else pad_token_id
        with eval_no_grad(self):
            enc, mask = self.model.encoder(input_ids, vis_inputs, attention_mask, task, no_padding)
            key_mask = None if mask is None else mask[:, 0, 0, :].contiguous()
            dec = self.model.decoder
            state = dec.init_cache(enc, key_mask, task, max_length, num_beams=int(num_beams))
            V = self.model.shared.weight.shape[0]
            head = _padded_head(self.model.shared.weight, enc.dtype)
            bias = self._logits_bias()

            def make_step(st):
                def step(tok, pos):
                    logits = F.linear(dec.step(tok, pos, st, task), head)
                    if bias is not None:
                        logits[:, :V] += bias[0].to(logits.dtype)
                    return logits
                return step
            if graph:
                gs = D.GenSettings(cfg.decoder_start_token_id, eos, int(pad), int(max_length), int(min_length),
                                   int(no_repeat_ngram_size), int(num_beams), float(length_penalty), bool(early_stopping), True)
                return D.graph_generate(self, state, make_step, V, cfg.decoder_attention_heads, head, gs, key_extra=(task,))[0]
            return D.generate(make_step(state), V, enc.shape[0], enc.device, state.key_rows, cfg.decoder_start_token_id, eos, pad,
                              max_length, min_length, no_repeat_ngram_size, int(num_beams), length_penalty, early_stopping,
                              force_eos=True)
```

vl-pet_amd/lmloss.py:

```python
from __future__ import annotations

from typing import Optional, Tuple

import torch
import torch.nn.functional as F

from . import _lib
from .functional import _io_dtype, _need_cuda, _stream, _timed


def _frozen_epoch():
    from . import functional as _VF
    return _VF.FROZEN_EPOCH


class _CeFn(torch.autograd.Function):
    @staticmethod
    def forward(ctx, logits, labels, V):
        lib = _lib.load()
        _need_cuda(logits, labels)
        N, ld = logits.shape
        io = _io_dtype(logits)
        lab = labels.contiguous()
        if lab.dtype != torch.int64:
            lab = lab.long()
        loss = torch.empty(N, dtype=torch.float32, device=logits.device)
        lse = torch.empty(N, dtype=torch.float32, device=logits.device)
        bad = _bad_counter(logits.device)
        rc = _timed("ce_fwd", N, lambda: lib.vlpet_ce_loss_fwd_checked(logits.data_ptr(), lab.data_ptr(), loss.data_ptr(), lse.data_ptr(),
                                                                       bad.data_ptr(), N, V, ld, io, _stream()))
        _lib.check(rc, "vlpet_ce_loss_fwd_checked")
        ctx.save_for_backward(logits, lab, lse)
        ctx.cfg = (V, io)
        return loss

    @staticmethod
    def backward(ctx, dloss):
        lib = _lib.load()
        logits, lab, lse = ctx.saved_tensors
        V, io = ctx.cfg
        N, ld = logits.shape
        g = dloss.contiguous().float()
        dlogits = torch.empty_like(logits)
        rc = _timed("ce_bwd", N, lambda: lib.vlpet_ce_loss_bwd(logits.data_ptr(), lab.data_ptr(), lse.data_ptr(), g.data_ptr(),
                                                               dlogits.data_ptr(), N, V, ld, io, _stream()))
        _lib.check(rc, "vlpet_ce_loss_bwd")
        return dlogits, None, None


def cross_entropy_rows(logits: torch.Tensor, labels: torch.Tensor, V: Optional[int] = None) -> torch.Tensor:
    if logits.dim() != 2 or not logits.is_contiguous():
        raise RuntimeError("vl-pet_amd: cross_entropy_rows needs contiguous [N, ld] logits")
    V = logits.shape[1] if V is None else int(V)
    if logits.shape[1] % 8 != 0:
        raise RuntimeError("vl-pet_amd: logits row stride must be a multiple of 8 (use lm_head_loss, which pads the head)")
    labels = labels.reshape(-1)
    if logits.shape[0] == 0:
        return logits.new_zeros(0, dtype=torch.float32) + 0.0 * logits.float().sum()
    _check_labels_once(labels, V)
    return _CeFn.apply(logits, labels, V)


CHECK_LABELS = "once"
_CHECKED = set()
_BAD = {}


def _bad_counter(device: torch.device) -> torch.Tensor:
    key = (device.type, device.index)
    t = _BAD.get(key)
    if t is None:
        t = _BAD[key] = torch.zeros(1, dtype=torch.int32, device=device)
    return t


def bad_label_count(device=None) -> int:
    ts = [t for k, t in _BAD.items() if device is None or k == (torch.device(device).type, torch.device(device).index)]
    return int(sum(int(t.item()) for t in ts))


def _check_labels_once(labels: torch.Tensor, V: int):
    if CHECK_LABELS == "never":
        return
    key = (V, labels.dtype, labels.device.type)
    if CHECK_LABELS == "once" and key in _CHECKED:
        return
    bad = (labels >= V) | ((labels < 0) & (labels != -100))
    if bool(bad.any()):
        raise IndexError(f"vl-pet_amd: label {int(labels[bad][0])} outside [0, {V}) (and not ignore_index -100)")
    _CHECKED.add(key)


def _padded_head(weight: torch.Tensor, dtype: torch.dtype) -> torch.Tensor:
    V, d = weight.shape
    Vp = (V + 7) // 8 * 8
    if weight.requires_grad:
        w = weight.to(dtype)
        return w if Vp == V else torch.cat([w, w.new_zeros(Vp - V, d)], 0)
    key = (weight.data_ptr(), weight._version, dtype, tuple(weight.shape), _frozen_epoch())
    hit = getattr(weight, "_vlpet_padded_head", None)
    if hit is not None and hit[0] == key:
        return hit[1]
    with torch.no_grad():
        wp = torch.zeros(Vp, d, dtype=dtype, device=weight.device)
        wp[:V].copy_(weight)
    weight._vlpet_padded_head = (key, wp)
    return wp


def lm_head_loss(h: torch.Tensor, weight: torch.Tensor, labels: torch.Tensor,
                 bias: Optional[torch.Tensor] = None) -> Tuple[torch.Tensor, torch.Tensor]:
    V = weight.shape[0]
    wp = _padded_head(weight, h.dtype)
    logits = F.linear(h, wp)
    if bias is not None and bool(bias.any()):
        logits = logits + F.pad(bias.to(h.dtype).reshape(-1), (0, wp.shape[0] - V))
    flat = logits.reshape(-1, wp.shape[0])
    loss = cross_entropy_rows(flat, labels, V)
    return loss.view(labels.shape), logits[..., :V]
```

vl-pet_amd/train.py:

```python
from __future__ import annotations

import collections
import math
import os
import random
from typing import Dict, List, Optional, Sequence

import torch
import torch.distributed as dist
import torch.nn as nn

TASK_BATCH = {"vqa": lambda b: b, "gqa": lambda b: int(b * 100 / 60), "nlvr": lambda b: int(b * 20 / 60),
              "caption": lambda b: int(b * 50 / 60),
              "tvqa": lambda b: b, "how2qa": lambda b: b, "tvc": lambda b: b, "yc2c": lambda b: b}
TEXT_LEN = {"vqa": 20, "gqa": 20, "nlvr": 20, "caption": 40, "tvqa": 600, "how2qa": 600, "tvc": 600, "yc2c": 600}
TARGET_LEN = {"vqa": 5, "gqa": 5, "nlvr": 2, "caption": 20, "tvqa": 3, "how2qa": 3, "tvc": 20, "yc2c": 20}
VIDEO_TASKS = ("tvqa", "how2qa", "tvc", "yc2c")
VIDEO_FRAMES = 64


def trainable_names(model: nn.Module, config) -> List[str]:
    names = []
    for n, p in model.named_parameters():
        p.requires_grad = False
    any_adapter = bool(config.use_encoder_adapter_down_multihead or
                       config.use_decoder_enc_attn_value_parallel_adapter_down_dim)
    any_gate = bool(config.use_encoder_adapter_gating_large_x_lowrank or
                    config.use_encoder_adapter_gating_small_xy_cat or
                    config.use_encoder_adapter_gating_middle_xy_add or
                    config.use_encoder_adapter_gating_middle_ia3_add)
    compacter = bool(getattr(config, "use_compacter", False))
    any_adapter = any_adapter or bool((config.use_adapter or compacter) and not (config.no_encoder_adapter and config.no_decoder_adapter))
    ac = getattr(config, "adapter_config", None)
    learn_phm = bool(getattr(ac, "learn_phm", True))
    norm_params = set()
    if getattr(config, "unfreeze_layer_norms", False):
        from .visual import T5LayerNorm
        norm_params = {id(p) for m in model.modules() if isinstance(m, (nn.LayerNorm, T5LayerNorm)) for p in m.parameters()}
    prompt_params = set()
    if getattr(config, "encoder_prompt_len", 0) > 0 or getattr(config, "decoder_prompt_len", 0) > 0:
        from .prompt import PromptController
        prompt_params = {id(p) for m in model.modules() if isinstance(m, PromptController) for p in m.parameters()}
    for n, p in model.named_parameters():
        on = id(p) in norm_params or id(p) in prompt_params
        if not config.freeze_vis_emb and "visual_embedding" in n:
            on = True
        if config.use_lora and ("lora" in n or "bias" in n):
            on = True
        if config.unfreeze_encoder_layer_norms and "encoder." in n and ("layer_norm" in n or "layernorm" in n):
            on = True
        if any_gate and "gating" in n:
            on = True
        if any_adapter and "adapter" in n:
            on = True
        if compacter and any_adapter and n == "phm_rule":
            on = True
        if compacter and not learn_phm and "phm_rule" in n:
            on = False
        if on:
            p.requires_grad = True
            names.append(n)
    return names


def weight_initialization(model: nn.Module, config):
    with torch.no_grad():
        for n, p in model.named_parameters():
            if config.use_encoder_multihead_up_zero_init and "adapter_multihead_up" in n:
                p.zero_()
            if config.use_encoder_gating_large_x_lowrank_up_zero_init and "adapter_gating_large_x_up" in n:
                p.zero_()
            if config.use_decoder_enc_vpa_up_zero_init and "attn_value_parallel_adapter" in n and "up_sampler" in n:
                p.zero_()
            if getattr(config, "use_encoder_gating_small_up_zero_init", False) and "adapter_gating_small_xy_cat" in n:
                p.zero_()
            if getattr(config, "use_encoder_gating_middle_up_zero_init", False) and "adapter_gating_middle_xy_add" in n:
                p.zero_()
            if getattr(config, "use_encoder_gating_middle_ia3_one_init", False) and "adapter_gating_middle_ia3_add" in n:
                p.fill_(1.0)
            if getattr(config, "use_encoder_gating_middle_ia3_zero_init", False) and "adapter_gating_middle_ia3_add" in n:
                p.zero_()


def cast_frozen(model: nn.Module, dtype: torch.dtype):
    for p in model.parameters():
        if not p.requires_grad and p.is_floating_point():
            p.data = p.data.to(dtype)
    for b in model.buffers():
        if b.is_floating_point():
            b.data = b.data.to(dtype)


def synthetic_batch(task: str, batch: int, config, device, gen: torch.Generator, feat_dtype=torch.float32, no_padding: bool = True):
    V = config.vocab_size - 200
    L, T = TEXT_LEN[task], TARGET_LEN[task]
    n_grid = 49
    ids = torch.randint(5, V, (batch, L), device=device, generator=gen)
    labels = torch.randint(5, V, (batch, T), device=device, generator=gen)
    if task in VIDEO_TASKS:
        feats = torch.randn(batch, VIDEO_FRAMES, int(config.feat_dim), device=device, generator=gen, dtype=feat_dtype)
        boxes = torch.zeros(batch, VIDEO_FRAMES, 4, device=device, dtype=feat_dtype)
        return dict(task=task, input_ids=ids, vis_inputs=(feats, boxes), labels=labels, scores=None, no_padding=no_padding)
    if task == "nlvr":
        feats = torch.randn(batch, 2 * n_grid, int(config.feat_dim), device=device, generator=gen, dtype=feat_dtype)
        boxes = torch.zeros(batch, 2 * n_grid, 4, device=device, dtype=feat_dtype)
        img = torch.cat([torch.zeros(n_grid, dtype=torch.long), torch.ones(n_grid, dtype=torch.long)])
        obj = torch.cat([torch.arange(n_grid), torch.arange(n_grid)])
        vis = (feats, boxes, img.to(device).unsqueeze(0).expand(batch, -1), obj.to(device).unsqueeze(0).expand(batch, -1))
    else:
        feats = torch.randn(batch, n_grid, int(config.feat_dim), device=device, generator=gen, dtype=feat_dtype)
        boxes = torch.zeros(batch, n_grid, 4, device=device, dtype=feat_dtype)
        vis = (feats, boxes)
    return dict(task=task, input_ids=ids, vis_inputs=vis, labels=labels,
                scores=torch.ones(batch, device=device), no_padding=no_padding)


def epoch_task_order(tasks: Sequence[str], steps_per_task: Dict[str, int], epoch: int) -> List[str]:
    order = []
    for t in tasks:
        order += [t] * steps_per_task[t]
    random.Random(epoch).shuffle(order)
    return order


def task_loss(per_token: torch.Tensor, labels: torch.Tensor, scores: Optional[torch.Tensor], task: str):
    mask = (labels != -100).float()
    if task in ("vqa", "gqa") or task in VIDEO_TASKS:
        loss = (per_token * mask).sum(1) / mask.sum(1).clamp(min=1)
        if scores is not None and task not in VIDEO_TASKS:
            loss = loss * scores
        return loss.mean()
    return (per_token * mask).sum() / mask.sum().clamp(min=1)


class GradSink:

    def __init__(self, owner: "FlatGrads", view: torch.Tensor, indices: Sequence[int]):
        self.owner, self.view, self.indices = owner, view, tuple(indices)
        self.epoch = -1

    def take(self) -> Optional[torch.Tensor]:
        if not self.owner.sinks_enabled:
            return None
        if self.epoch == self.owner.epoch:
            from . import functional as VF
            VF.flush_reduces()
            if self.owner.dp:
                raise RuntimeError("vl-pet_amd: a parameter with a direct-write gradient slot was used twice in one "
                                   "backward under data parallelism; build FlatGrads(sinks=False) for such models")
            return None
        self.epoch = self.owner.epoch
        return self.view

    def done(self):
        for i in self.indices:
            self.owner._ready(i)


def _flat_order(named):
    import re

    def readiness(n):
        if ".decoder." in n:
            return 0
        if "visual_embedding" in n or "layernorm_embedding" in n:
            return 2
        return 1
    pat = re.compile(r"(.*adapter_multihead_down)\.(\d+)\.(weight|bias)$")
    first_seen = {}
    keyed = []
    for pos, (n, p) in enumerate(named):
        mm = pat.match(n)
        if mm:
            g = mm.group(1)
            first_seen.setdefault(g, pos)
            keyed.append(((readiness(n), first_seen[g], 0 if mm.group(3) == "weight" else 1, int(mm.group(2))), n, p))
        else:
            keyed.append(((readiness(n), pos, 0, 0), n, p))
    keyed.sort(key=lambda t: t[0])
    return [(n, p) for _, n, p in keyed]


def _has_per_task_params(names, params) -> bool:
    import re
    pat = re.compile(r"(.*\.(?:adapters|lora_As|lora_Bs|prompts))\.([^.]+)(\..*)?$")
    seen = {}
    for n in names:
        m = pat.match(n)
        if m:
            seen.setdefault((m.group(1), m.group(3) or ""), set()).add(m.group(2))
    return any(len(v) > 1 for v in seen.values())


class FlatGrads:

    def __init__(self, model: nn.Module, world_size: int = 1, n_buckets: int = 3, process_group=None,
                 flatten_params: bool = False, sinks: bool = False, force_collectives: bool = False):
        named = _flat_order([(n, p) for n, p in model.named_parameters() if p.requires_grad])
        self.names = [n for n, _ in named]
        self.params = [p for _, p in named]
        total = sum(p.numel() for p in self.params)
        total_pad = (total + 3) // 4 * 4
        dev = self.params[0].device
        self.total = total
        self.flat = torch.zeros(total_pad, dtype=torch.float32, device=dev)
        self.world_size = world_size
        self.dp = world_size > 1 or force_collectives
        self.group = process_group
        self.epoch = 0
        self.defer = False
        self.sinks_enabled = bool(sinks)
        off = 0
        self.slices = []
        for p in self.params:
            n = p.numel()
            p.grad = self.flat[off:off + n].view_as(p)
            self.slices.append((off, off + n))
            off += n
        self.flat_p = None
        self.flat_p_io = None
        self.io_epoch = -1
        if flatten_params:
            self.flat_p = torch.zeros(total_pad, dtype=torch.float32, device=dev)
            for p, (a, b) in zip(self.params, self.slices):
                self.flat_p[a:b].copy_(p.data.reshape(-1).float())
                p.data = self.flat_p[a:b].view_as(p)
        self.bucket_of = []
        self.buckets = []
        n_buckets = max(1, min(n_buckets, len(self.params)))
        target = total / n_buckets
        start, cur = 0, 0
        for i, (a, b) in enumerate(self.slices):
            self.bucket_of.append(len(self.buckets))
            cur = b
            if cur - start >= target and len(self.buckets) < n_buckets - 1:
                self.buckets.append((start, cur))
                start = cur
        self.buckets.append((start, total))
        self.bucket_count = [0] * len(self.buckets)
        for bidx in self.bucket_of:
            self.bucket_count[bidx] += 1
        self._pending = [0] * len(self.buckets)
        self._ready_epoch = [-1] * len(self.params)
        self._handles = []
        self._hooks = []
        self.per_task = _has_per_task_params(self.names, self.params)
        if self.dp or self.per_task:
            for i, p in enumerate(self.params):
                self._hooks.append(p.register_post_accumulate_grad_hook(self._make_hook(i)))
        if sinks:
            self._attach_sinks()

    def _attach_sinks(self):
        import re
        pat = re.compile(r"(.*adapter_multihead_down)\.(\d+)\.(weight|bias)$")
        groups: Dict[tuple, List[int]] = {}
        for i, n in enumerate(self.names):
            mm = pat.match(n)
            if mm:
                groups.setdefault((mm.group(1), mm.group(3)), []).append(i)
        in_group = set()
        for (_, kind), idx in groups.items():
            idx.sort()
            a, b = self.slices[idx[0]][0], self.slices[idx[-1]][1]
            contiguous = all(self.slices[idx[k]][1] == self.slices[idx[k + 1]][0] for k in range(len(idx) - 1))
            if not contiguous:
                continue
            first = self.params[idx[0]]
            rows = sum(self.params[i].shape[0] for i in idx)
            view = self.flat[a:b].view(rows, *first.shape[1:]) if kind == "weight" else self.flat[a:b]
            first._vlpet_block_sink = GradSink(self, view, idx)
            in_group.update(idx)
        for i, p in enumerate(self.params):
            if i not in in_group:
                a, b = self.slices[i]
                p._vlpet_sink = GradSink(self, self.flat[a:b].view_as(p), [i])

    def _ready(self, i):
# ... 421 lines not shown
```

Measured before the change: 29310.

## Fuse encoder/decoder input assembly and task-loss reduction into HIP kernels

Adds fused kernels that build encoder and decoder inputs in one pass: embedding gather, scaling, positional add, layernorm, vision concat, key-mask and dropout, with a backward that produces vision grads and layernorm partials. It also adds a fused masked task-loss reduction kernel with its own backward, which train.py enables by default. The aim is to cut the many small PyTorch elementwise and reduction launches and the intermediate tensors around the model's inputs and loss. The risks are rounding differences from mimicking bf16 intermediate rounding, and whether model code actually calls the input-assembly path.

```diff
diff --git a/include/vlpet_hip.h b/include/vlpet_hip.h
--- a/include/vlpet_hip.h
+++ b/include/vlpet_hip.h
@@ -249,6 +249,22 @@
                                     float p, uint64_t seed, int io_dtype, vlpet_stream_t stream);
 int vlpet_prefix_concat_dropout_bwd(const void* dx, void* dpre, void* da, void* dv, float* ws, int64_t B, int P, int La, int Lv, int d,
                                     float p, uint64_t seed, int io_dtype, vlpet_stream_t stream);
+int vlpet_inputs_applies(int d, int io_dtype, int gb_dtype);
+int vlpet_decoder_inputs_fwd(const int64_t* labels, const void* E, const void* P, const void* gamma, const void* beta, void* x,
+                             uint8_t* keep_out, int64_t B, int T, int d, int64_t V, int pos_rows, int pad_id, int start_id,
+                             float scale, float eps, float p, uint64_t seed, int gb_dtype, int io_dtype, vlpet_stream_t stream);
+int vlpet_encoder_inputs_fwd(const int64_t* ids, const void* E, const void* P, const void* gamma, const void* beta, const void* vis,
+                             void* x, uint8_t* key_mask, float* stats, uint8_t* keep_out, int64_t B, int La, int Lv, int d, int64_t V,
+                             int pos_rows, int pad_id, float scale, float eps, float p, uint64_t seed, int gb_dtype, int io_dtype,
+                             vlpet_stream_t stream);
+int vlpet_encoder_inputs_chunks(int64_t text_rows);
+int vlpet_encoder_inputs_bwd(const void* dx, const int64_t* ids, const void* E, const void* P, const float* stats, void* dvis,
+                             float* dgb_partials, int64_t B, int La, int Lv, int d, int64_t V, int pos_rows, float scale, float p,
+                             uint64_t seed, int io_dtype, vlpet_stream_t stream);
+
+int vlpet_task_loss_fwd(const float* per_token, const int64_t* labels, const float* scores, float* loss, float* w, int64_t B, int T,
+                        int per_sample, vlpet_stream_t stream);
+int vlpet_task_loss_bwd(const float* dloss, const float* w, float* dper_token, int64_t B, int T, vlpet_stream_t stream);
 
 int vlpet_ce_loss_fwd(const void* logits, const int64_t* labels, float* loss, float* lse, int64_t N, int V, int ld,
                       int io_dtype, vlpet_stream_t stream);
diff --git a/vl-pet_amd/_lib.py b/vl-pet_amd/_lib.py
--- a/vl-pet_amd/_lib.py
+++ b/vl-pet_amd/_lib.py
@@ -133,6 +133,16 @@
     "vlpet_prefix_concat_ws_bytes": (c_size_t, [c_int64, c_int, c_int]),
     "vlpet_prefix_concat_dropout_fwd": (c_int, [c_void_p] * 4 + [c_int64, c_int, c_int, c_int, c_int, c_float, c_uint64, c_int, c_void_p]),
     "vlpet_prefix_concat_dropout_bwd": (c_int, [c_void_p] * 5 + [c_int64, c_int, c_int, c_int, c_int, c_float, c_uint64, c_int, c_void_p]),
+    "vlpet_inputs_applies": (c_int, [c_int, c_int, c_int]),
+    "vlpet_decoder_inputs_fwd": (c_int, [c_void_p] * 7 + [c_int64, c_int, c_int, c_int64, c_int, c_int, c_int, c_float, c_float, c_float,
+                                         c_uint64, c_int, c_int, c_void_p]),
+    "vlpet_encoder_inputs_fwd": (c_int, [c_void_p] * 10 + [c_int64, c_int, c_int, c_int, c_int64, c_int, c_int, c_float, c_float, c_float,
+                                         c_uint64, c_int, c_int, c_void_p]),
+    "vlpet_encoder_inputs_chunks": (c_int, [c_int64]),
+    "vlpet_encoder_inputs_bwd": (c_int, [c_void_p] * 7 + [c_int64, c_int, c_int, c_int, c_int64, c_int, c_float, c_float, c_uint64, c_int,
+                                         c_void_p]),
+    "vlpet_task_loss_fwd": (c_int, [c_void_p] * 5 + [c_int64, c_int, c_int, c_void_p]),
+    "vlpet_task_loss_bwd": (c_int, [c_void_p] * 3 + [c_int64, c_int, c_void_p]),
     "vlpet_attn_fwd_kv": (c_int, [c_void_p] * 8 + [c_int] * 8 + [c_float, c_float, c_uint64, c_void_p]),
     "vlpet_attn_bwd_kv": (c_int, [c_void_p] * 12 + [c_int] * 8 + [c_float, c_float, c_uint64, c_void_p]),
     "vlpet_attn_long_fwd": (c_int, [c_void_p] * 7 + [c_int] * 8 + [c_float, c_void_p]),
diff --git a/vl-pet_amd/csrc/api.hip b/vl-pet_amd/csrc/api.hip
--- a/vl-pet_amd/csrc/api.hip
+++ b/vl-pet_amd/csrc/api.hip
@@ -7,7 +7,7 @@
 #include <stdio.h>
 #include <vector>
 
-#define VLPET_VERSION 680
+#define VLPET_VERSION 690
 #define VLPET_VERSION_R3 300
 #define VLPET_VERSION_R2 221
 
@@ -1469,6 +1469,88 @@
     return herr(launch_prefix_cat(c, true, io_dtype == VLPET_F32, (hipStream_t)stream));
 }
 
+extern "C" int vlpet_inputs_applies(int d, int io_dtype, int gb_dtype) {
+    if (d <= 0 || d % 8 != 0 || d > INPUTS_MAX_D || !dtype_ok(io_dtype) || !dtype_ok(gb_dtype)) return 0;
+    return (io_dtype == VLPET_F32 && gb_dtype != VLPET_F32) ? 0 : 1;
+}
+static inline bool aligned8(const void* p) { return (reinterpret_cast<uintptr_t>(p) & 7) == 0; }
+static inline bool aligned4(const void* p) { return (reinterpret_cast<uintptr_t>(p) & 3) == 0; }
+static int inputs_common(int64_t B, int rows_len, int d, int64_t V, int pos_rows, int pad_id, float p, int gb_dtype, int io_dtype) {
+    if (B <= 0 || rows_len <= 0 || d <= 0 || d % 8 != 0 || d > INPUTS_MAX_D || V <= 0 || !(p >= 0.f && p < 1.f)) return VLPET_E_SHAPE;
+    if (pos_rows < rows_len + 2 || pad_id < 0 || pad_id >= V) return VLPET_E_SHAPE;
+    if (!dtype_ok(io_dtype) || !dtype_ok(gb_dtype) || (io_dtype == VLPET_F32 && gb_dtype != VLPET_F32)) return VLPET_E_DTYPE;
+    return 0;
+}
+static EmbedNormArgs embed_norm_args(const void* E, const void* P, const void* gamma, const void* beta, void* x, uint8_t* keep_out, int64_t V,
+                                     int d, float scale, float eps, float p, uint64_t seed) {
+    EmbedNormArgs n{};
+    n.E = E; n.P = P; n.gamma = gamma; n.beta = beta; n.gb_vec = aligned16(gamma) && aligned16(beta); n.x = x; n.keep_out = keep_out; n.V = V; n.d = d; n.scale = scale; n.eps = eps;
+    n.thr = tail_thr(p); n.keep_scale = n.thr ? 1.0f / (1.0f - p) : 1.0f; n.seed = seed; n.seed_ctr = g_seed_ctr.load();
+    return n;
+}
+extern "C" int vlpet_decoder_inputs_fwd(const int64_t* labels, const void* E, const void* P, const void* gamma, const void* beta, void* x,
+                                        uint8_t* keep_out, int64_t B, int T, int d, int64_t V, int pos_rows, int pad_id, int start_id,
+                                        float scale, float eps, float p, uint64_t seed, int gb_dtype, int io_dtype, vlpet_stream_t stream) {
+    if (!labels || !E || !P || !gamma || !beta || !x) return VLPET_E_NULL;
+    if (int rc = inputs_common(B, T, d, V, pos_rows, pad_id, p, gb_dtype, io_dtype)) return rc;
+    if (start_id < 0 || start_id >= V || !(eps >= 0.f)) return VLPET_E_SHAPE;
+    if (!aligned16(E) || !aligned16(P) || !aligned4(gamma) || !aligned4(beta) || !aligned16(x) || !aligned8(keep_out)) return VLPET_E_ALIGN;
+    DecInputsArgs a{};
+    a.n = embed_norm_args(E, P, gamma, beta, x, keep_out, V, d, scale, eps, p, seed);
+    a.labels = labels; a.B = B; a.T = T; a.pad_id = pad_id; a.start_id = start_id;
+    return herr(launch_decoder_inputs(a, io_dtype == VLPET_F32, gb_dtype == VLPET_F32, (hipStream_t)stream));
+}
+extern "C" int vlpet_encoder_inputs_fwd(const int64_t* ids, const void* E, const void* P, const void* gamma, const void* beta, const void* vis,
+                                        void* x, uint8_t* key_mask, float* stats, uint8_t* keep_out, int64_t B, int La, int Lv, int d, int64_t V,
+                                        int pos_rows, int pad_id, float scale, float eps, float p, uint64_t seed, int gb_dtype, int io_dtype,
+                                        vlpet_stream_t stream) {
+    if (!ids || !E || !P || !gamma || !beta || !vis || !x) return VLPET_E_NULL;
+    if (int rc = inputs_common(B, La, d, V, pos_rows, pad_id, p, gb_dtype, io_dtype)) return rc;
+    if (Lv <= 0 || !(eps >= 0.f)) return VLPET_E_SHAPE;
+    if (!aligned16(E) || !aligned16(P) || !aligned4(gamma) || !aligned4(beta) || !aligned16(vis) || !aligned16(x) || !aligned8(keep_out)
+        || !aligned8(stats))
+        return VLPET_E_ALIGN;
+    EncInputsArgs a{};
+    a.n = embed_norm_args(E, P, gamma, beta, x, keep_out, V, d, scale, eps, p, seed);
+    a.ids = ids; a.vis = vis; a.key_mask = key_mask; a.stats = stats; a.B = B; a.La = La; a.Lv = Lv; a.pad_id = pad_id;
+    return herr(launch_encoder_inputs_fwd(a, io_dtype == VLPET_F32, gb_dtype == VLPET_F32, (hipStream_t)stream));
+}
+extern "C" int vlpet_encoder_inputs_chunks(int64_t text_rows) {
+    if (text_rows <= 0) return 0;
+    int rpc, nc;
+    enc_inputs_split(text_rows, &rpc, &nc);
+    return nc;
+}
+extern "C" int vlpet_encoder_inputs_bwd(const void* dx, const int64_t* ids, const void* E, const void* P, const float* stats, void* dvis,
+                                        float* dgb_partials, int64_t B, int La, int Lv, int d, int64_t V, int pos_rows, float scale, float p,
+                                        uint64_t seed, int io_dtype, vlpet_stream_t stream) {
+    if (!dx || (!dvis && !dgb_partials) || (dgb_partials && (!ids || !E || !P || !stats))) return VLPET_E_NULL;
+    if (int rc = inputs_common(B, La, d, V, pos_rows, 0, p, io_dtype, io_dtype)) return rc;
+    if (Lv <= 0) return VLPET_E_SHAPE;
+    if (!aligned16(dx) || !aligned16(dvis) || !aligned16(dgb_partials) || !aligned16(E) || !aligned16(P) || !aligned8(stats)) return VLPET_E_ALIGN;
+    EncInputsArgs a{};
+    a.n = embed_norm_args(E, P, nullptr, nullptr, nullptr, nullptr, V, d, scale, 0.f, p, seed);
+    a.ids = ids; a.stats = const_cast<float*>(stats); a.dx = dx; a.dvis = dvis; a.dgb = dgb_partials; a.B = B; a.La = La; a.Lv = Lv;
+    enc_inputs_split(B * (int64_t)La, &a.rows_per_chunk, &a.chunks);
+    return herr(launch_encoder_inputs_bwd(a, io_dtype == VLPET_F32, (hipStream_t)stream));
+}
+
+extern "C" int vlpet_task_loss_fwd(const float* per_token, const int64_t* labels, const float* scores, float* loss, float* w, int64_t B, int T,
+                                   int per_sample, vlpet_stream_t stream) {
+    if (!per_token || !labels || !loss || !w) return VLPET_E_NULL;
+    if (B <= 0 || T <= 0 || (scores && !per_sample)) return VLPET_E_SHAPE;
+    TaskLossArgs a{};
+    a.per_token = per_token; a.labels = labels; a.scores = scores; a.loss = loss; a.w = w; a.B = B; a.T = T; a.per_sample = per_sample ? 1 : 0;
+    return herr(launch_task_loss(a, false, (hipStream_t)stream));
+}
+extern "C" int vlpet_task_loss_bwd(const float* dloss, const float* w, float* dper_token, int64_t B, int T, vlpet_stream_t stream) {
+    if (!dloss || !w || !dper_token) return VLPET_E_NULL;
+    if (B <= 0 || T <= 0) return VLPET_E_SHAPE;
+    TaskLossArgs a{};
+    a.dloss = dloss; a.w = const_cast<float*>(w); a.dpt = dper_token; a.B = B; a.T = T;
+    return herr(launch_task_loss(a, true, (hipStream_t)stream));
+}
+
 extern "C" int vlpet_act_dropout_bwd(const void* dy, const void* x, void* dx, int64_t n, int act, float p, uint64_t seed,
                                      int io_dtype, vlpet_stream_t stream) {
     int rc = act_common(n, act, p, io_dtype);
diff --git a/vl-pet_amd/csrc/input_assembly.hip b/vl-pet_amd/csrc/input_assembly.hip
--- /dev/null
+++ b/vl-pet_amd/csrc/input_assembly.hip
@@ -0,0 +1,324 @@
+#include "common.h"
+#include "kernels.h"
+#include "rng.h"
+#include "vec8.h"
+
+template <typename T> __device__ __forceinline__ float round_to(float f) { return (float)(T)f; }
+
+template <typename T> __device__ __forceinline__ void load8f(const void* p, int64_t g, float (&o)[8]);
+template <> __device__ __forceinline__ void load8f<__bf16>(const void* p, int64_t g, float (&o)[8]) {
+    const bf16x8 v = reinterpret_cast<const bf16x8*>(p)[g];
+#pragma unroll
+    for (int j = 0; j < 8; ++j) o[j] = (float)v[j];
+}
+template <> __device__ __forceinline__ void load8f<float>(const void* p, int64_t g, float (&o)[8]) {
+    const f32x4 a = reinterpret_cast<const f32x4*>(p)[2 * g], b = reinterpret_cast<const f32x4*>(p)[2 * g + 1];
+#pragma unroll
+    for (int j = 0; j < 4; ++j) { o[j] = a[j]; o[4 + j] = b[j]; }
+}
+
+__device__ __forceinline__ float wave_sum(float v) {
+#pragma unroll
+    for (int o = 32; o >= 1; o >>= 1) v += __shfl_xor(v, o, 64);
+    return v;
+}
+
+template <typename IO>
+__device__ __forceinline__ void embed_group(const EmbedNormArgs& n, int64_t id, int t, int g, float (&v)[8]) {
+    const int gpr = n.d >> 3;
+    float e[8] = {0.f, 0.f, 0.f, 0.f, 0.f, 0.f, 0.f, 0.f}, pe[8];
+    if (id >= 0 && id < n.V) load8f<IO>(n.E, id * gpr + g, e);
+    load8f<IO>(n.P, (int64_t)(2 + t) * gpr + g, pe);
+#pragma unroll
+    for (int j = 0; j < 8; ++j) v[j] = round_to<IO>(round_to<IO>(e[j] * n.scale) + pe[j]);
+}
+
+template <typename IO, typename GB, int NG, bool DROP>
+__device__ __forceinline__ void embed_norm_row(const EmbedNormArgs& n, int64_t id, int t, int64_t row, uint64_t seed, int lane, float* stats) {
+    const int gpr = n.d >> 3;
+    const float inv_d = 1.0f / (float)n.d;
+    float v[NG][8];
+    float s = 0.f;
+#pragma unroll
+    for (int u = 0; u < NG; ++u) {
+        const int g = lane + 64 * u;
+#pragma unroll
+        for (int j = 0; j < 8; ++j) v[u][j] = 0.f;
+        if (g < gpr) {
+            embed_group<IO>(n, id, t, g, v[u]);
+#pragma unroll
+            for (int j = 0; j < 8; ++j) s += v[u][j];
+        }
+    }
+    const float mean = wave_sum(s) * inv_d;
+    float q = 0.f;
+#pragma unroll
+    for (int u = 0; u < NG; ++u)
+        if (lane + 64 * u < gpr) {
+#pragma unroll
+            for (int j = 0; j < 8; ++j) { const float c = v[u][j] - mean; q += c * c; }
+        }
+    const float rstd = 1.0f / sqrtf(wave_sum(q) * inv_d + n.eps);
+    if (stats != nullptr && lane == 0) { stats[0] = mean; stats[1] = rstd; }
+#pragma unroll
+    for (int u = 0; u < NG; ++u) {
+        const int g = lane + 64 * u;
+        if (g >= gpr) continue;
+        float gam[8], bet[8];
+        if (n.gb_vec) {
+            load8f<GB>(n.gamma, g, gam);
+            load8f<GB>(n.beta, g, bet);
+        } else {
+#pragma unroll
+            for (int j = 0; j < 8; ++j) {
+                gam[j] = (float)reinterpret_cast<const GB*>(n.gamma)[8 * g + j];
+                bet[j] = (float)reinterpret_cast<const GB*>(n.beta)[8 * g + j];
+            }
+        }
+        const int64_t xg = row * gpr + g;
+        uint32_t bits = 0xffu;
+        if constexpr (DROP) bits = keep8(xg, seed, n.thr);
+        Vec8<IO> o;
+#pragma unroll
+        for (int j = 0; j < 8; ++j) {
+            const float y = round_to<IO>(round_to<IO>(gam[j]) * (rstd * (v[u][j] - mean)) + round_to<IO>(bet[j]));
+            o.set(j, ((bits >> j) & 1u) ? y * n.keep_scale : 0.f);
+        }
+        o.store(n.x, xg);
+        if (n.keep_out != nullptr) drop_export8(n.keep_out, xg << 3, bits);
+    }
+}
+
+template <typename IO, typename GB, int NG, bool DROP>
+__global__ __launch_bounds__(256) void decoder_inputs_kernel(DecInputsArgs a) {
+    const int lane = threadIdx.x & 63;
+    const int64_t rows = a.B * (int64_t)a.T;
+    const int64_t nw = (int64_t)gridDim.x * 4;
+    const uint64_t seed = DROP ? vlpet_eff_seed(a.n.seed, a.n.seed_ctr) : 0;
+    for (int64_t row = (int64_t)blockIdx.x * 4 + (threadIdx.x >> 6); row < rows; row += nw) {
+        const int64_t b = row / a.T;
+        const int t = (int)(row - b * a.T);
+        int64_t id = t == 0 ? (int64_t)a.start_id : a.labels[row - 1];
+        if (id == -100) id = a.pad_id;
+        embed_norm_row<IO, GB, NG, DROP>(a.n, id, t, row, seed, lane, nullptr);
+    }
+}
+
+template <typename IO, typename GB, int NG, bool DROP>
+__global__ __launch_bounds__(256) void encoder_inputs_fwd_kernel(EncInputsArgs a) {
+    const int lane = threadIdx.x & 63, gpr = a.n.d >> 3, L = a.La + a.Lv;
+    const int64_t rows = a.B * (int64_t)L;
+    const int64_t nw = (int64_t)gridDim.x * 4;
+    const uint64_t seed = DROP ? vlpet_eff_seed(a.n.seed, a.n.seed_ctr) : 0;
+    for (int64_t row = (int64_t)blockIdx.x * 4 + (threadIdx.x >> 6); row < rows; row += nw) {
+        const int64_t b = row / L;
+        const int t = (int)(row - b * L);
+        if (t < a.La) {
+            const int64_t tr = b * a.La + t;
+            const int64_t id = a.ids[tr];
+            if (a.key_mask != nullptr && lane == 0) a.key_mask[row] = id != a.pad_id ? 1 : 0;
+            embed_norm_row<IO, GB, NG, DROP>(a.n, id, t, row, seed, lane, a.stats != nullptr ? a.stats + 2 * tr : nullptr);
+            continue;
+        }
+        if (a.key_mask != nullptr && lane == 0) a.key_mask[row] = 1;
+        const int64_t vrow = b * a.Lv + (t - a.La);
+        for (int g = lane; g < gpr; g += 64) {
+            const int64_t xg = row * gpr + g;
+            uint32_t bits = 0xffu;
+            if constexpr (DROP) bits = keep8(xg, seed, a.n.thr);
+            Vec8<IO> in, o;
+            in.load(a.vis, vrow * gpr + g);
+#pragma unroll
+            for (int j = 0; j < 8; ++j) o.set(j, ((bits >> j) & 1u) ? in.get(j) * a.n.keep_scale : 0.f);
+            o.store(a.n.x, xg);
+            if (a.n.keep_out != nullptr) drop_export8(a.n.keep_out, xg << 3, bits);
+        }
+    }
+}
+
+void enc_inputs_split(int64_t text_rows, int* rows_per_chunk, int* chunks) {
+    const int64_t r = (text_rows + ENC_INPUTS_MAX_CHUNKS - 1) / ENC_INPUTS_MAX_CHUNKS;
+    *rows_per_chunk = (int)r;
+    *chunks = (int)((text_rows + r - 1) / r);
+}
+
+template <typename IO, int NG, bool DROP>
+__global__ __launch_bounds__(256) void encoder_inputs_bwd_kernel(EncInputsArgs a, int n_stream) {
+    const int gpr = a.n.d >> 3, L = a.La + a.Lv;
+    const uint64_t seed = DROP ? vlpet_eff_seed(a.n.seed, a.n.seed_ctr) : 0;
+    if ((int)blockIdx.x < n_stream) {
+        const int64_t groups = a.B * (int64_t)a.Lv * gpr;
+        const int64_t stride = (int64_t)n_stream * blockDim.x;
+        for (int64_t s0 = (int64_t)blockIdx.x * blockDim.x + threadIdx.x; s0 < groups; s0 += 2 * stride) {
+            const bool two = s0 + stride < groups;
+            int64_t xg[2];
+            Vec8<IO> in[2];
+#pragma unroll
+            for (int u = 0; u < 2; ++u) {
+                if (u == 1 && !two) break;
+                const int64_t s = s0 + u * stride;
+                const int64_t vrow = s / gpr;
+                const int col = (int)(s - vrow * gpr);
+                const int64_t b = vrow / a.Lv;
+                const int t = (int)(vrow - b * a.Lv);
+                xg[u] = (b * L + a.La + t) * (int64_t)gpr + col;
+                in[u].load(a.dx, xg[u]);
+            }
+#pragma unroll
+            for (int u = 0; u < 2; ++u) {
+                if (u == 1 && !two) break;
+                uint32_t bits = 0xffu;
+                if constexpr (DROP) bits = keep8(xg[u], seed, a.n.thr);
+                Vec8<IO> o;
+#pragma unroll
+                for (int j = 0; j < 8; ++j) o.set(j, ((bits >> j) & 1u) ? in[u].get(j) * a.n.keep_scale : 0.f);
+                o.store(a.dvis, s0 + u * stride);
+            }
+        }
+        return;
+    }
+    extern __shared__ __attribute__((aligned(16))) float enc_sh[];
+    constexpr int RU = 2;
+    const int lane = threadIdx.x & 63, wave = threadIdx.x >> 6, d = a.n.d;
+    const int chunk = (int)blockIdx.x - n_stream;
+    const int64_t text_rows = a.B * (int64_t)a.La;
+    const int64_t c0 = (int64_t)chunk * a.rows_per_chunk;
+    const int64_t c1 = c0 + a.rows_per_chunk < text_rows ? c0 + a.rows_per_chunk : text_rows;
+    const int64_t q = (c1 - c0 + 3) / 4;
+    const int64_t r0 = c0 + wave * q < c1 ? c0 + wave * q : c1;
+    const int64_t r1 = r0 + q < c1 ? r0 + q : c1;
+    float ag[NG][8], ab[NG][8];
+#pragma unroll
+    for (int k = 0; k < NG; ++k)
+#pragma unroll
+        for (int j = 0; j < 8; ++j) ag[k][j] = ab[k][j] = 0.f;
+    for (int64_t r = r0; r < r1; r += RU) {
+        Vec8<IO> in[RU][NG];
+        float v[RU][NG][8], mean[RU], rstd[RU];
+        int64_t xrow[RU];
+#pragma unroll
+        for (int u = 0; u < RU; ++u) {
+            if (r + u >= r1) break;
+            const int64_t tr = r + u, b = tr / a.La;
+            const int t = (int)(tr - b * a.La);
+            const int64_t id = a.ids[tr];
+            xrow[u] = (b * L + t) * (int64_t)gpr;
+            mean[u] = a.stats[2 * tr];
+            rstd[u] = a.stats[2 * tr + 1];
+#pragma unroll
+            for (int k = 0; k < NG; ++k) {
+                const int g = lane + 64 * k;
+                if (g >= gpr) break;
+                in[u][k].load(a.dx, xrow[u] + g);
+                embed_group<IO>(a.n, id, t, g, v[u][k]);
+            }
+        }
+#pragma unroll
+        for (int u = 0; u < RU; ++u) {
+            if (r + u >= r1) break;
+#pragma unroll
+            for (int k = 0; k < NG; ++k) {
+                const int g = lane + 64 * k;
+                if (g >= gpr) break;
+                uint32_t bits = 0xffu;
+                if constexpr (DROP) bits = keep8(xrow[u] + g, seed, a.n.thr);
+#pragma unroll
+                for (int j = 0; j < 8; ++j) {
+                    const float dy = ((bits >> j) & 1u) ? round_to<IO>(in[u][k].get(j) * a.n.keep_scale) : 0.f;
+                    ag[k][j] += dy * ((v[u][k][j] - mean[u]) * rstd[u]);
+                    ab[k][j] += dy;
+                }
+            }
+        }
+    }
+    if (wave > 0) {
+        float* s = enc_sh + (int64_t)(wave - 1) * 2 * d;
+#pragma unroll
+        for (int k = 0; k < NG; ++k) {
+            const int g = lane + 64 * k;
+            if (g >= gpr) break;
+#pragma unroll
+            for (int j = 0; j < 8; ++j) { s[8 * g + j] = ag[k][j]; s[d + 8 * g + j] = ab[k][j]; }
+        }
+    }
+    __syncthreads();
+    if (wave > 0) return;
+    float* part = a.dgb + (int64_t)chunk * 2 * d;
+#pragma unroll
+    for (int k = 0; k < NG; ++k) {
+        const int g = lane + 64 * k;
+        if (g >= gpr) break;
+        for (int w = 0; w < 3; ++w) {
+            const float* s = enc_sh + (int64_t)w * 2 * d;
+#pragma unroll
+            for (int j = 0; j < 8; ++j) { ag[k][j] += s[8 * g + j]; ab[k][j] += s[d + 8 * g + j]; }
+        }
+        f32x4* pg = reinterpret_cast<f32x4*>(part) + 2 * g;
+        f32x4* pb = reinterpret_cast<f32x4*>(part + d) + 2 * g;
+        pg[0] = f32x4{ag[k][0], ag[k][1], ag[k][2], ag[k][3]}; pg[1] = f32x4{ag[k][4], ag[k][5], ag[k][6], ag[k][7]};
+        pb[0] = f32x4{ab[k][0], ab[k][1], ab[k][2], ab[k][3]}; pb[1] = f32x4{ab[k][4], ab[k][5], ab[k][6], ab[k][7]};
+    }
+}
+
+static unsigned row_blocks(int64_t rows) {
+    int64_t blocks = (rows + 3) / 4;
+    if (blocks > 256 * 16) blocks = 256 * 16;
+    return (unsigned)blocks;
+}
+
+template <typename IO, typename GB, int NG>
+static hipError_t launch_dec_inputs_ng(const DecInputsArgs& a, hipStream_t stream) {
+    const dim3 grid(row_blocks(a.B * (int64_t)a.T)), blk(256);
+    if (a.n.thr != 0) hipLaunchKernelGGL((decoder_inputs_kernel<IO, GB, NG, true>), grid, blk, 0, stream, a);
+    else hipLaunchKernelGGL((decoder_inputs_kernel<IO, GB, NG, false>), grid, blk, 0, stream, a);
+    return hipGetLastError();
+}
+template <typename IO, typename GB, int NG>
+static hipError_t launch_enc_inputs_ng(const EncInputsArgs& a, hipStream_t stream) {
+    const dim3 grid(row_blocks(a.B * (int64_t)(a.La + a.Lv))), blk(256);
+    if (a.n.thr != 0) hipLaunchKernelGGL((encoder_inputs_fwd_kernel<IO, GB, NG, true>), grid, blk, 0, stream, a);
+    else hipLaunchKernelGGL((encoder_inputs_fwd_kernel<IO, GB, NG, false>), grid, blk, 0, stream, a);
+    return hipGetLastError();
+}
+
+#define VLPET_INPUTS_DISPATCH(f, a, d, io_fp32, gb_fp32, stream)                                                          \
+    do {                                                                                                                  \
+        if ((d) > INPUTS_MAX_D) return hipErrorInvalidValue;                                                              \
+        const bool wide = (d) > 64 * 8 * 2;                                                                               \
+        if (io_fp32) return wide ? f<float, float, 4>(a, stream) : f<float, float, 2>(a, stream);                         \
+        if (gb_fp32) return wide ? f<__bf16, float, 4>(a, stream) : f<__bf16, float, 2>(a, stream);                       \
+        return wide ? f<__bf16, __bf16, 4>(a, stream) : f<__bf16, __bf16, 2>(a, stream);                                  \
+    } while (0)
+
+hipError_t launch_decoder_inputs(const DecInputsArgs& a, int io_fp32, int gb_fp32, hipStream_t stream) {
+    if (a.B <= 0 || a.T <= 0) return hipSuccess;
+    VLPET_INPUTS_DISPATCH(launch_dec_inputs_ng, a, a.n.d, io_fp32, gb_fp32, stream);
+}
+hipError_t launch_encoder_inputs_fwd(const EncInputsArgs& a, int io_fp32, int gb_fp32, hipStream_t stream) {
+    if (a.B <= 0) return hipSuccess;
+    VLPET_INPUTS_DISPATCH(launch_enc_inputs_ng, a, a.n.d, io_fp32, gb_fp32, stream);
+}
+#undef VLPET_INPUTS_DISPATCH
+
+template <typename IO, int NG>
+static hipError_t launch_enc_inputs_bwd_ng(const EncInputsArgs& a, hipStream_t stream) {
+    const int gpr = a.n.d >> 3;
+    int64_t n_stream = 0, n_part = 0;
+    if (a.dvis != nullptr) {
+        n_stream = (a.B * (int64_t)a.Lv * gpr + 511) / 512;
+        if (n_stream > 256 * 16) n_stream = 256 * 16;
+    }
+    if (a.dgb != nullptr) n_part = a.chunks;
+    if (n_stream + n_part == 0) return hipSuccess;
+    const dim3 grid((unsigned)(n_stream + n_part)), blk(256);
+    const size_t lds = n_part ? (size_t)3 * 2 * a.n.d * sizeof(float) : 0;
+    if (a.n.thr != 0) hipLaunchKernelGGL((encoder_inputs_bwd_kernel<IO, NG, true>), grid, blk, lds, stream, a, (int)n_stream);
+    else hipLaunchKernelGGL((encoder_inputs_bwd_kernel<IO, NG, false>), grid, blk, lds, stream, a, (int)n_stream);
+    return hipGetLastError();
+}
+hipError_t launch_encoder_inputs_bwd(const EncInputsArgs& a, int io_fp32, hipStream_t stream) {
+    if (a.n.d > INPUTS_MAX_D) return hipErrorInvalidValue;
+    const bool wide = a.n.d > 64 * 8 * 2;
+    if (io_fp32) return wide ? launch_enc_inputs_bwd_ng<float, 4>(a, stream) : launch_enc_inputs_bwd_ng<float, 2>(a, stream);
+    return wide ? launch_enc_inputs_bwd_ng<__bf16, 4>(a, stream) : launch_enc_inputs_bwd_ng<__bf16, 2>(a, stream);
+}
diff --git a/vl-pet_amd/csrc/kernels.h b/vl-pet_amd/csrc/kernels.h
--- a/vl-pet_amd/csrc/kernels.h
+++ b/vl-pet_amd/csrc/kernels.h
@@ -376,6 +376,46 @@
 void prefix_cat_split(int64_t B, int* cs, int* nc);
 hipError_t launch_prefix_cat(const PrefixCatArgs& c, bool bwd, int io_fp32, hipStream_t stream);
 
+#define INPUTS_MAX_D 2048
+struct EmbedNormArgs {
+    const void* E; const void* P;
+    const void* gamma; const void* beta;
+    int gb_vec;
+    void* x;
+    uint8_t* keep_out;
+    int64_t V; int d;
+    float scale, eps;
+    uint32_t thr; float keep_scale; uint64_t seed; const uint64_t* seed_ctr;
+};
+struct DecInputsArgs {
+    EmbedNormArgs n;
+    const int64_t* labels;
+    int64_t B; int T, pad_id, start_id;
+};
+hipError_t launch_decoder_inputs(const DecInputsArgs& a, int io_fp32, int gb_fp32, hipStream_t stream);
+#define ENC_INPUTS_MAX_CHUNKS 1024
+struct EncInputsArgs {
+    EmbedNormArgs n;
+    const int64_t* ids;
+    const void* vis;
+    uint8_t* key_mask;
+    float* stats;
+    const void* dx; void* dvis;
+    float* dgb;
+    int64_t B; int La, Lv, pad_id, rows_per_chunk, chunks;
+};
+void enc_inputs_split(int64_t text_rows, int* rows_per_chunk, int* chunks);
+hipError_t launch_encoder_inputs_fwd(const EncInputsArgs& a, int io_fp32, int gb_fp32, hipStream_t stream);
+hipError_t launch_encoder_inputs_bwd(const EncInputsArgs& a, int io_fp32, hipStream_t stream);
+
+struct TaskLossArgs {
+    const float* per_token; const int64_t* labels; const float* scores;
+    float* loss; float* w;
+    const float* dloss; float* dpt;
+    int64_t B; int T, per_sample;
+};
+hipError_t launch_task_loss(const TaskLossArgs& a, bool bwd, hipStream_t stream);
+
 struct CeArgs {
     const void* logits;
     const int64_t* labels;
diff --git a/vl-pet_amd/csrc/task_loss.hip b/vl-pet_amd/csrc/task_loss.hip
--- /dev/null
+++ b/vl-pet_amd/csrc/task_loss.hip
@@ -0,0 +1,84 @@
+#include "common.h"
+#include "kernels.h"
+
+#define TASK_LOSS_THREADS 1024
+
+__device__ __forceinline__ double wave_sum_f64(double v) {
+#pragma unroll
+    for (int o = 32; o >= 1; o >>= 1) v += __shfl_xor(v, o, 64);
+    return v;
+}
+__device__ __forceinline__ double block_sum_f64(double v, double* sh) {
+    v = wave_sum_f64(v);
+    __syncthreads();
+    if ((threadIdx.x & 63) == 0) sh[threadIdx.x >> 6] = v;
+    __syncthreads();
+    double s = 0.0;
+#pragma unroll
+    for (int k = 0; k < TASK_LOSS_THREADS / 64; ++k) s += sh[k];
+    return s;
+}
+
+__global__ __launch_bounds__(TASK_LOSS_THREADS) void task_loss_fwd_kernel(TaskLossArgs a) {
+    __shared__ double sh[TASK_LOSS_THREADS / 64];
+    if (a.per_sample) {
+        const float inv_b = 1.0f / (float)a.B;
+        double acc = 0.0;
+        for (int64_t b = threadIdx.x; b < a.B; b += TASK_LOSS_THREADS) {
+            const float* p = a.per_token + b * a.T;
+            const int64_t* l = a.labels + b * a.T;
+            double s = 0.0;
+            int n = 0;
+            for (int t = 0; t < a.T; ++t) {
+                const bool m = l[t] != -100;
+                s += (double)(p[t] * (m ? 1.0f : 0.0f));
+                n += m ? 1 : 0;
+            }
+            const float cnt = (float)(n > 1 ? n : 1);
+            float g = inv_b;
+            double ls = s / (double)cnt;
+            if (a.scores != nullptr) {
+                const float sc = a.scores[b];
+                ls *= (double)sc;
+                g *= sc;
+            }
+            acc += ls;
+            g = g / cnt;
+            float* w = a.w + b * a.T;
+            for (int t = 0; t < a.T; ++t) w[t] = g * (l[t] != -100 ? 1.0f : 0.0f);
+        }
+        const double tot = block_sum_f64(acc, sh);
+        if (threadIdx.x == 0) *a.loss = (float)(tot / (double)a.B);
+        return;
+    }
+    const int64_t n_el = a.B * a.T;
+    double s = 0.0, n = 0.0;
+    for (int64_t i = threadIdx.x; i < n_el; i += TASK_LOSS_THREADS) {
+        const bool m = a.labels[i] != -100;
+        s += (double)(a.per_token[i] * (m ? 1.0f : 0.0f));
+        n += m ? 1.0 : 0.0;
+    }
+    const double tot = block_sum_f64(s, sh);
+    const double cnt_d = block_sum_f64(n, sh);
+    const float cnt = cnt_d > 1.0 ? (float)cnt_d : 1.0f;
+    if (threadIdx.x == 0) *a.loss = (float)(tot / (double)cnt);
+    const float g = 1.0f / cnt;
+    for (int64_t i = threadIdx.x; i < n_el; i += TASK_LOSS_THREADS) a.w[i] = g * (a.labels[i] != -100 ? 1.0f : 0.0f);
+}
+
+__global__ __launch_bounds__(256) void task_loss_bwd_kernel(TaskLossArgs a) {
+    const int64_t n_el = a.B * a.T;
+    const float g = *a.dloss;
+    for (int64_t i = (int64_t)blockIdx.x * blockDim.x + threadIdx.x; i < n_el; i += (int64_t)gridDim.x * blockDim.x) a.dpt[i] = g * a.w[i];
+}
+
+hipError_t launch_task_loss(const TaskLossArgs& a, bool bwd, hipStream_t stream) {
+    if (!bwd) {
+        hipLaunchKernelGGL(task_loss_fwd_kernel, dim3(1), dim3(TASK_LOSS_THREADS), 0, stream, a);
+        return hipGetLastError();
+    }
+    int64_t blocks = (a.B * a.T + 255) / 256;
+    if (blocks > 256 * 16) blocks = 256 * 16;
+    hipLaunchKernelGGL(task_loss_bwd_kernel, dim3((unsigned)blocks), dim3(256), 0, stream, a);
+    return hipGetLastError();
+}
diff --git a/vl-pet_amd/host/bart.py b/vl-pet_amd/host/bart.py
--- a/vl-pet_amd/host/bart.py
+++ b/vl-pet_amd/host/bart.py
@@ -423,6 +423,9 @@
         return super().forward(torch.arange(2, L + 2, device=device))
 
 
+FUSE_INPUT_ASSEMBLY = True
+
+
 class JointEncoder(nn.Module):
     def __init__(self, config, embed_tokens):
         super().__init__()
@@ -447,10 +450,23 @@
         if getattr(self, "prompt_modules", None) is not None:
             return self._forward_prompted(input_ids, vis_inputs, attention_mask, task, no_padding)
         B, L = input_ids.shape
+        vis = None
+        if attention_mask is None and self._fused_inputs_ok(input_ids):
+            from ..inputs import encoder_inputs, encoder_inputs_apply
+            E, P = self.embed_tokens.weight, self.embed_positions.weight
+            vis = self.visual_embedding(*unpack_vis_inputs(vis_inputs, self.downsample, E.dtype)).to(E.dtype)
+            if encoder_inputs_apply(input_ids, vis, E, P, self.layernorm_embedding):
+                x, km = encoder_inputs(input_ids, vis, E, P, self.layernorm_embedding, self.config.pad_token_id, self.embed_scale,
+                                       self.dropout, self.training, key_mask=not no_padding)
+                mask = None if km is None else km[:, None, None, :]
+                for layer in self.layers:
+                    x = layer(x, mask, task)
+                return x, mask
         if attention_mask is None and not no_padding:
             attention_mask = input_ids.ne(self.config.pad_token_id)
         x = self.embed_tokens(input_ids) * self.embed_scale + self.embed_positions(L, input_ids.device)
-        vis = self.visual_embedding(*unpack_vis_inputs(vis_inputs, self.downsample, x.dtype)).to(x.dtype)
+        if vis is None:
+            vis = self.visual_embedding(*unpack_vis_inputs(vis_inputs, self.downsample, x.dtype)).to(x.dtype)
         if self.config.share_vis_lang_layer_norm:
             x = self.layernorm_embedding(torch.cat([x, vis], dim=1))
             x = F.dropout(x, p=self.dropout, training=self.training)
@@ -465,6 +481,12 @@
         for layer in self.layers:
             x = layer(x, mask, task)
         return x, mask
+
+    def _fused_inputs_ok(self, input_ids) -> bool:
+        if not FUSE_INPUT_ASSEMBLY or self.config.share_vis_lang_layer_norm or type(self.embed_tokens) is not nn.Embedding:
+            return False
+        from ..inputs import tables_apply
+        return tables_apply(input_ids, self.embed_tokens.weight, self.embed_positions.weight, self.layernorm_embedding)
 
     def _forward_prompted(self, input_ids, vis_inputs, attention_mask, task, no_padding):
         B, L = input_ids.shape
@@ -500,10 +522,21 @@
         self.layers = nn.ModuleList([BartDecoderLayer(config) for _ in range(config.decoder_layers)])
         self.layernorm_embedding = HostLayerNorm(d)
 
-    def forward(self, input_ids, enc, enc_mask=None, task=None):
-        B, L = input_ids.shape
-        x = self.embed_tokens(input_ids) * self.embed_scale + self.embed_positions(L, input_ids.device)
-        x = F.dropout(self.layernorm_embedding(x), p=self.dropout, training=self.training)
+    def inputs_from_labels(self, labels, pad_id, start_id):
+        if not FUSE_INPUT_ASSEMBLY or type(self.embed_tokens) is not nn.Embedding:
+            return None
+        from ..inputs import decoder_inputs, decoder_inputs_apply
+        E, P = self.embed_tokens.weight, self.embed_positions.weight
+        if not decoder_inputs_apply(labels, E, P, self.layernorm_embedding):
+            return None
+        x = decoder_inputs(labels, E, P, self.layernorm_embedding, pad_id, start_id, self.embed_scale, 0.0, False)
+        return F.dropout(x, p=self.dropout, training=self.training)
+
+    def forward(self, input_ids, enc, enc_mask=None, task=None, x=None):
+        if x is None:
+            B, L = input_ids.shape
+            x = self.embed_tokens(input_ids) * self.embed_scale + self.embed_positions(L, input_ids.device)
+            x = F.dropout(self.layernorm_embedding(x), p=self.dropout, training=self.training)
         n = len(self.layers)
         fused_keys = self._cross_keys_ok(enc, enc_mask)
         encs = VF.fanout(enc, n + (1 if fused_keys else 0))
@@ -593,8 +626,12 @@
     def forward(self, input_ids, vis_inputs, labels, task, attention_mask=None, no_padding=False):
         cfg = self.config
         enc, mask = self.model.encoder(input_ids, vis_inputs, attention_mask, task, no_padding)
-        dec_in = shift_tokens_right(labels, cfg.pad_token_id, cfg.decoder_start_token_id)
-        h = self.model.decoder(dec_in, enc, mask, task)
+        x0 = self.model.decoder.inputs_from_labels(labels, cfg.pad_token_id, cfg.decoder_start_token_id)
+        if x0 is not None:
+            h = self.model.decoder(None, enc, mask, task, x=x0)
+        else:
+            dec_in = shift_tokens_right(labels, cfg.pad_token_id, cfg.decoder_start_token_id)
+            h = self.model.decoder(dec_in, enc, mask, task)
         return lm_loss(h, self.model.shared.weight, labels, self._logits_bias())
 
     def generate(self, input_ids, vis_inputs, task, attention_mask=None, max_length=20, min_length=0, no_repeat_ngram_size=0,
diff --git a/vl-pet_amd/inputs.py b/vl-pet_amd/inputs.py
--- /dev/null
+++ b/vl-pet_amd/inputs.py
@@ -0,0 +1,137 @@
+from __future__ import annotations
+
+from typing import Optional
+
+import torch
+
+from . import _lib
+from .functional import _io_dtype, _need_cuda, _ptr, _stream, _timed, grad_slot, reduce_partials
+from .tail import _draw_seed
+
+
+def tables_apply(ids: torch.Tensor, E: torch.Tensor, P: torch.Tensor, norm) -> bool:
+    if not (ids.is_cuda and ids.dtype == torch.int64 and ids.dim() == 2 and ids.numel() > 0):
+        return False
+    if not (E.is_cuda and P.is_cuda and E.dim() == 2 and P.dim() == 2 and E.dtype == P.dtype and E.dtype in (torch.bfloat16, torch.float32)
+            and E.shape[1] == P.shape[1] and E.is_contiguous() and P.is_contiguous() and E.data_ptr() % 16 == 0 and P.data_ptr() % 16 == 0):
+        return False
+    if torch.is_grad_enabled() and (E.requires_grad or P.requires_grad):
+        return False
+    d = E.shape[1]
+    if not isinstance(norm, torch.nn.LayerNorm) or norm.weight is None or norm.bias is None or tuple(norm.normalized_shape) != (d,):
+        return False
+    w, b = norm.weight, norm.bias
+    if not (w.is_cuda and b.is_cuda and w.dtype == b.dtype and w.dtype in (torch.float32, E.dtype) and w.is_contiguous() and b.is_contiguous()
+            and w.data_ptr() % 4 == 0 and b.data_ptr() % 4 == 0):
+        return False
+    if ids.shape[1] + 2 > P.shape[0]:
+        return False
+    return bool(_lib.load().vlpet_inputs_applies(d, _io_dtype(E), _io_dtype(w)))
+
+
+def decoder_inputs_apply(labels: torch.Tensor, E: torch.Tensor, P: torch.Tensor, norm) -> bool:
+    if not tables_apply(labels, E, P, norm):
+        return False
+    return not (torch.is_grad_enabled() and (norm.weight.requires_grad or norm.bias.requires_grad))
+
+
+def encoder_inputs_apply(ids: torch.Tensor, vis: torch.Tensor, E: torch.Tensor, P: torch.Tensor, norm) -> bool:
+    if not tables_apply(ids, E, P, norm):
+        return False
+    return (vis.is_cuda and vis.dim() == 3 and vis.dtype == E.dtype and vis.shape[0] == ids.shape[0] and vis.shape[1] > 0
+            and vis.shape[2] == E.shape[1])
+
+
+def decoder_inputs(labels: torch.Tensor, E: torch.Tensor, P: torch.Tensor, norm, pad_id: int, start_id: int, scale: float = 1.0,
+                   p: float = 0.0, training: bool = False, seed: Optional[int] = None, return_mask: bool = False):
+    lib = _lib.load()
+    _need_cuda(labels, E, P)
+    B, T = labels.shape
+    V, d = E.shape
+    pe = float(p) if training else 0.0
+    if seed is None:
+        seed = _draw_seed() if pe > 0.0 else 0
+    lab = labels.contiguous()
+    w, b = norm.weight.detach(), norm.bias.detach()
+    x = torch.empty(B, T, d, dtype=E.dtype, device=E.device)
+    mask = torch.empty(B, T, d, dtype=torch.uint8, device=E.device) if return_mask else None
+    rc = _timed("dec_inputs_fwd", B * T, lambda: lib.vlpet_decoder_inputs_fwd(
+        lab.data_ptr(), E.data_ptr(), P.data_ptr(), w.data_ptr(), b.data_ptr(), x.data_ptr(), _ptr(mask), B, T, d, V, P.shape[0], int(pad_id),
+        int(start_id), float(scale), float(norm.eps), pe, int(seed), _io_dtype(w), _io_dtype(E), _stream()))
+    _lib.check(rc, "vlpet_decoder_inputs_fwd")
+    return (x, mask) if return_mask else x
+
+
+class _EncoderInputsFn(torch.autograd.Function):
+    @staticmethod
+    def forward(ctx, vis, gamma, beta, ids, E, P, eps, pad_id, scale, p, seed, want_km, want_mask):
+        lib = _lib.load()
+        _need_cuda(vis, gamma, beta, ids, E, P)
+        B, La = ids.shape
+        V, d = E.shape
+        Lv = vis.shape[1]
+        L = La + Lv
+        io = _io_dtype(E)
+        idc, vc = ids.contiguous(), vis.contiguous()
+        dev = E.device
+        x = torch.empty(B, L, d, dtype=E.dtype, device=dev)
+        km = torch.empty(B, L, dtype=torch.bool, device=dev) if want_km else None
+        mask = torch.empty(B, L, d, dtype=torch.uint8, device=dev) if want_mask else None
+        train_ln = ctx.needs_input_grad[1] or ctx.needs_input_grad[2]
+        stats = torch.empty(B * La, 2, dtype=torch.float32, device=dev) if train_ln else None
+        rc = _timed("enc_inputs_fwd", B * L, lambda: lib.vlpet_encoder_inputs_fwd(
+            idc.data_ptr(), E.data_ptr(), P.data_ptr(), gamma.data_ptr(), beta.data_ptr(), vc.data_ptr(), x.data_ptr(), _ptr(km), _ptr(stats),
+            _ptr(mask), B, La, Lv, d, V, P.shape[0], int(pad_id), float(scale), float(eps), float(p), seed, _io_dtype(gamma), io, _stream()))
+        _lib.check(rc, "vlpet_encoder_inputs_fwd")
+        ctx.save_for_backward(idc, E, P, stats, gamma, beta)
+        ctx.cfg = (B, La, Lv, d, V, float(scale), float(p), seed, io, E.dtype)
+        outs = [x]
+        for t in (km, mask):
+            if t is not None:
+                ctx.mark_non_differentiable(t)
+                outs.append(t)
+        return tuple(outs) if len(outs) > 1 else x
+
+    @staticmethod
+    def backward(ctx, dx, *unused):
+        lib = _lib.load()
+        idc, E, P, stats, gamma, beta = ctx.saved_tensors
+        B, La, Lv, d, V, scale, p, seed, io, dtype = ctx.cfg
+        none = (None,) * 13
+        want_v = ctx.needs_input_grad[0]
+        train_ln = stats is not None and (ctx.needs_input_grad[1] or ctx.needs_input_grad[2])
+        if not want_v and not train_ln:
+            return none
+        dxc = dx.contiguous()
+        if dxc.dtype != dtype:
+            dxc = dxc.to(dtype)
+        dvis = torch.empty(B, Lv, d, dtype=dtype, device=dx.device) if want_v else None
+        part = None
+        if train_ln:
+            part = torch.empty(lib.vlpet_encoder_inputs_chunks(B * La), 2, d, dtype=torch.float32, device=dx.device)
+        rc = _timed("enc_inputs_bwd", B * (La + Lv), lambda: lib.vlpet_encoder_inputs_bwd(
+            dxc.data_ptr(), idc.data_ptr(), E.data_ptr(), P.data_ptr(), _ptr(stats), _ptr(dvis), _ptr(part), B, La, Lv, d, V, P.shape[0], scale,
+            p, seed, io, _stream()))
+        _lib.check(rc, "vlpet_encoder_inputs_bwd")
+        dgamma = dbeta = None
+        if train_ln:
+            sg = grad_slot(gamma, (d,)) if ctx.needs_input_grad[1] else None
+            sb = grad_slot(beta, (d,)) if ctx.needs_input_grad[2] else None
+            reduce_partials(part, part.shape[0], d, sg.t if sg else None, sb.t if sb else None,
+                            deferrable=(sg is None or sg.sunk) and (sb is None or sb.sunk))
+            dgamma = sg.finish() if sg else None
+            dbeta = sb.finish() if sb else None
+        return (dvis, dgamma, dbeta) + (None,) * 10
+
+
+def encoder_inputs(ids: torch.Tensor, vis: torch.Tensor, E: torch.Tensor, P: torch.Tensor, norm, pad_id: int, scale: float = 1.0,
+                   p: float = 0.0, training: bool = False, key_mask: bool = True, seed: Optional[int] = None, return_mask: bool = False):
+    pe = float(p) if training else 0.0
+    if seed is None:
+        seed = _draw_seed() if pe > 0.0 else 0
+    out = _EncoderInputsFn.apply(vis, norm.weight, norm.bias, ids, E, P, float(norm.eps), int(pad_id), float(scale), pe, int(seed),
+                                 bool(key_mask), bool(return_mask))
+    out = list(out) if isinstance(out, tuple) else [out]
+    x = out.pop(0)
+    km = out.pop(0) if key_mask else None
+    return (x, km, out.pop(0)) if return_mask else (x, km)
diff --git a/vl-pet_amd/lmloss.py b/vl-pet_amd/lmloss.py
--- a/vl-pet_amd/lmloss.py
+++ b/vl-pet_amd/lmloss.py
@@ -91,6 +91,46 @@
     _CHECKED.add(key)
 
 
+class _TaskLossFn(torch.autograd.Function):
+
+    @staticmethod
+    def forward(ctx, per_token, labels, scores, per_sample):
+        lib = _lib.load()
+        _need_cuda(per_token, labels, scores)
+        B, T = per_token.shape
+        pt, lab = per_token.contiguous(), labels.contiguous()
+        sc = None if scores is None else scores.contiguous()
+        loss = torch.empty((), dtype=torch.float32, device=pt.device)
+        w = torch.empty(B, T, dtype=torch.float32, device=pt.device)
+        rc = _timed("task_loss_fwd", B, lambda: lib.vlpet_task_loss_fwd(pt.data_ptr(), lab.data_ptr(), None if sc is None else sc.data_ptr(),
+                                                                        loss.data_ptr(), w.data_ptr(), B, T, int(per_sample), _stream()))
+        _lib.check(rc, "vlpet_task_loss_fwd")
+        ctx.save_for_backward(w)
+        return loss
+
+    @staticmethod
+    def backward(ctx, dloss):
+        lib = _lib.load()
+        (w,) = ctx.saved_tensors
+        B, T = w.shape
+        g = dloss.contiguous().float()
+        dpt = torch.empty_like(w)
+        rc = _timed("task_loss_bwd", B, lambda: lib.vlpet_task_loss_bwd(g.data_ptr(), w.data_ptr(), dpt.data_ptr(), B, T, _stream()))
+        _lib.check(rc, "vlpet_task_loss_bwd")
+        return dpt, None, None, None
+
+
+def task_loss_applies(per_token: torch.Tensor, labels: torch.Tensor, scores: Optional[torch.Tensor]) -> bool:
+    return (per_token.is_cuda and per_token.dtype == torch.float32 and per_token.dim() == 2 and per_token.numel() > 0
+            and labels.is_cuda and labels.dtype == torch.int64 and labels.shape == per_token.shape
+            and (scores is None or (scores.is_cuda and scores.dtype == torch.float32 and scores.shape == per_token.shape[:1]
+                                    and not scores.requires_grad)))
+
+
+def task_loss_reduce(per_token: torch.Tensor, labels: torch.Tensor, scores: Optional[torch.Tensor], per_sample: bool) -> torch.Tensor:
+    return _TaskLossFn.apply(per_token, labels, scores, bool(per_sample))
+
+
 def _padded_head(weight: torch.Tensor, dtype: torch.dtype) -> torch.Tensor:
     V, d = weight.shape
     Vp = (V + 7) // 8 * 8
diff --git a/vl-pet_amd/train.py b/vl-pet_amd/train.py
--- a/vl-pet_amd/train.py
+++ b/vl-pet_amd/train.py
@@ -123,7 +123,16 @@
     return order
 
 
+FUSE_TASK_LOSS = True
+
+
 def task_loss(per_token: torch.Tensor, labels: torch.Tensor, scores: Optional[torch.Tensor], task: str):
+    if FUSE_TASK_LOSS and per_token.is_cuda:
+        from . import lmloss
+        per_sample = task in ("vqa", "gqa") or task in VIDEO_TASKS
+        sc = scores if per_sample and task not in VIDEO_TASKS else None
+        if lmloss.task_loss_applies(per_token, labels, sc):
+            return lmloss.task_loss_reduce(per_token, labels, sc, per_sample)
     mask = (labels != -100).float()
     if task in ("vqa", "gqa") or task in VIDEO_TASKS:
         loss = (per_token * mask).sum(1) / mask.sum(1).clamp(min=1)
```

After: 29590, median of 6. No clear change (+0.9%).
